# lukasvst/dm-vio

Hardware: NVIDIA H100
Metric: point-residuals/sec per GN iter (7 KF, 2000 pts, 640x480) (higher is better)
Workload: dtype f32

## Files before the change

### dm-vio_b200/capi.py

```python
import ctypes as C
import os

import numpy as np

_HERE = os.path.dirname(os.path.abspath(__file__))
LIB_PATH = os.environ.get("DMVIO_B200_LIB") or os.path.join(_HERE, "libdmvio_b200.so")
_LIB = None

f32p = np.ctypeslib.ndpointer(dtype=np.float32, flags="C_CONTIGUOUS")
f64p = np.ctypeslib.ndpointer(dtype=np.float64, flags="C_CONTIGUOUS")
i32p = np.ctypeslib.ndpointer(dtype=np.int32, flags="C_CONTIGUOUS")
vp = C.c_void_p

MAX_FRAMES = 8
PRECALC_FLOATS = 32


class DmvError(RuntimeError):
    pass


class BAConfig(C.Structure):
    _fields_ = [("w", C.c_int), ("h", C.c_int), ("max_frames", C.c_int), ("max_points", C.c_int), ("device", C.c_int), ("chunk_points", C.c_int)]


class BAParams(C.Structure):
    _fields_ = [("huberTH", C.c_float), ("outlierTHSumComponent", C.c_float), ("affineOptModeA", C.c_float), ("affineOptModeB", C.c_float)]


class BAState(C.Structure):
    _fields_ = [("calib", C.c_float * 8), ("precalc", vp), ("frameEnergyTH", vp), ("idepth", vp), ("idepth_zero", vp)]


class BALinResult(C.Structure):
    _fields_ = [("energy", C.c_double), ("n_in", C.c_int), ("n_oob", C.c_int), ("n_outlier", C.c_int)]


class BAActivateArgs(C.Structure):
    _fields_ = [("n", C.c_int)] + [(k, C.c_void_p) for k in ("host", "u", "v", "color8", "weights8", "energyTH", "idepth_min", "idepth_max", "RT")] + \
               [("minObs", C.c_int)] + [(k, C.c_void_p) for k in ("status", "idepth", "res_state")]


class BAMargArgs(C.Structure):
    _fields_ = [("n", C.c_int32), ("point", C.c_void_p), ("adHTdeltaF", C.c_void_p), ("cDeltaF", C.c_float * 4), ("idepthFixPriorMargFac", C.c_float)] + \
               [(k, C.c_void_p) for k in ("M", "Mb", "Msc", "Mbsc", "resInM", "ngoodRes", "res_toZeroF", "isLinearized")]


class IPPoints(C.Structure):
    _fields_ = [("n", C.c_int)] + [(k, C.c_void_p) for k in ("u", "v", "color8", "weights8", "gradH4", "energyTH", "idepth_min", "idepth_max", "quality",
                                                              "lastTraceStatus", "lastTraceUV2", "lastTracePixelInterval")]


class BABatch:

    def __init__(self, bas):
        self.L = lib()
        self.bas = list(bas)
        n = len(self.bas)
        self._harr = (C.c_void_p * n)(*[b.h for b in self.bas])
        h = C.c_void_p()
        check(self.L.dmv_ba_batch_create(self._harr, n, C.byref(h)))
        self.h = h

    def _args(self, xs, states):
        n = len(self.bas)
        self._xs = [None if x is None else _c(x, np.float64) for x in (xs or [None] * n)]
        self._sts = [b._state(*st) for b, st in zip(self.bas, states)]
        xarr = (C.c_void_p * n)(*[None if x is None else x.ctypes.data for x in self._xs])
        sarr = (C.c_void_p * n)(*[C.addressof(st) for st in self._sts])
        return xarr, sarr

    def gn_step(self, xs, states):
        n = len(self.bas)
        xarr, sarr = self._args(xs, states)
        res = (BALinResult * n)()
        sums = np.zeros(3 * n)
        check(self.L.dmv_ba_batch_gn_step(self.h, xarr, sarr, res, sums.ctypes.data))
        return [dict(energy=r.energy, n_in=r.n_in, n_oob=r.n_oob, n_outlier=r.n_outlier, sums=sums[3 * i:3 * i + 3]) for i, r in enumerate(res)]

    def bench(self, xs, states, iters=100, warmup=5):
        n = len(self.bas)
        xarr, sarr = self._args(xs, states)
        e2e, ker = C.c_double(0), C.c_double(0)
        check(self.L.dmv_ba_batch_bench(self.h, self._harr, n, xarr, sarr, max(1, warmup), C.byref(e2e), C.byref(ker)))
        check(self.L.dmv_ba_batch_bench(self.h, self._harr, n, xarr, sarr, iters, C.byref(e2e), C.byref(ker)))
        return ker.value, e2e.value, None

    def close(self):
        if self.h:
            self.L.dmv_ba_batch_destroy(self.h)
            self.h = None

    def __del__(self):
        try:
            self.close()
        except Exception:
            pass


class CTConfig(C.Structure):
    _fields_ = [("w", C.c_int), ("h", C.c_int), ("levels", C.c_int), ("max_points", C.c_int), ("device", C.c_int)]


class CIEvalArgs(C.Structure):
    _fields_ = [("level", C.c_int), ("RKi", C.c_float * 9), ("t_d", C.c_double * 3), ("t_log", C.c_double * 3), ("r2new_aff", C.c_float * 2),
                ("huberTH", C.c_float), ("alphaK", C.c_float), ("alphaW", C.c_float), ("couplingWeight", C.c_float),
                ("weightZeroPriorX", C.c_double), ("weightZeroPriorY", C.c_double),
                ("idepth_new", C.c_void_p), ("isGood", C.c_void_p), ("energy2", C.c_void_p), ("iR", C.c_void_p),
                ("isGood_new", C.c_void_p), ("energy_new2", C.c_void_p), ("maxstep", C.c_void_p), ("lastHessian_new", C.c_void_p),
                ("JbBuffer_new10", C.c_void_p)]


class CIEvalResult(C.Structure):
    _fields_ = [("H", C.c_float * 64), ("b", C.c_float * 8), ("Hsc", C.c_float * 64), ("bsc", C.c_float * 8), ("res3", C.c_float * 3),
                ("alphaOpt", C.c_float), ("n_good_new", C.c_int)]


SYMBOLS = [
    "dmv_last_error", "dmv_version", "dmv_device_count",
    "dmv_ba_create", "dmv_ba_destroy", "dmv_ba_set_params", "dmv_ba_default_params", "dmv_ba_upload_frame", "dmv_ba_upload_image", "dmv_ba_adopt_frame",
    "dmv_ba_set_window", "dmv_ba_set_points", "dmv_ba_set_residuals", "dmv_ba_set_adjoints", "dmv_ba_set_state", "dmv_ba_linearize",
    "dmv_ba_get_residual_outputs", "dmv_ba_get_target_energies", "dmv_ba_apply_res", "dmv_ba_accumulate", "dmv_ba_get_point_outputs", "dmv_ba_get_solve_HdiF",
    "dmv_ba_resubstitute", "dmv_ba_backup_points", "dmv_ba_restore_points", "dmv_ba_get_idepth", "dmv_ba_gn_step", "dmv_nccl_unique_id",
    "dmv_ba_comm_init", "dmv_ba_activate_points", "dmv_ba_marginalize_points", "dmv_ba_drop_residuals", "dmv_ba_reset_oob", "dmv_ba_p2p_export", "dmv_ba_p2p_import", "dmv_ba_last_timing", "dmv_ba_bench_device", "dmv_ba_kernel_launch_count", "dmv_ba_io_bytes", "dmv_ba_set_timing", "dmv_ba_bench_e2e",
    "dmv_ba_batch_create", "dmv_ba_batch_destroy", "dmv_ba_batch_gn_step", "dmv_ba_batch_set_timing", "dmv_ba_batch_last_kernel_ms", "dmv_ba_batch_bench",
    "dmv_ct_create", "dmv_ct_destroy", "dmv_ct_set_K", "dmv_ct_set_ref", "dmv_ct_make_coarse_depth", "dmv_ct_get_ref", "dmv_ct_upload_new", "dmv_ct_upload_new_image", "dmv_ct_set_huber",
    "dmv_ci_create", "dmv_ci_destroy", "dmv_ci_set_K", "dmv_ci_upload_first", "dmv_ci_upload_new", "dmv_ci_set_points", "dmv_ci_calc_res_and_gs", "dmv_ci_kernel_launch_count",
    "dmv_ct_calc_res_gs", "dmv_ct_track", "dmv_ip_default_settings", "dmv_ct_init_points", "dmv_ct_trace_points", "dmv_ct_trace_points_multi", "dmv_ct_set_timing", "dmv_ct_last_timing", "dmv_ct_kernel_launch_count", "dmv_ct_last_point_evaluations",
]


def lib():
    global _LIB
    if _LIB is None:
        if not os.path.exists(LIB_PATH):
            raise DmvError(f"{LIB_PATH} is missing: build it with `make -C dm-vio_b200` (python -c 'import __graft_entry__ as g; g.build()')")
        L = C.CDLL(LIB_PATH)
        L.dmv_last_error.restype = C.c_char_p
        L.dmv_version.restype = C.c_char_p
        L.dmv_ba_create.argtypes = [C.POINTER(BAConfig), C.POINTER(vp)]
        L.dmv_ba_destroy.argtypes = [vp]
        L.dmv_ba_set_params.argtypes = [vp, C.POINTER(BAParams)]
        L.dmv_ba_default_params.argtypes = [C.POINTER(BAParams)]
        L.dmv_ba_upload_frame.argtypes = [vp, C.c_int, f32p]
        L.dmv_ba_upload_image.argtypes = [vp, C.c_int, f32p]
        L.dmv_ba_set_window.argtypes = [vp, C.c_int, vp]
        L.dmv_ba_set_points.argtypes = [vp, C.c_int, i32p, f32p, f32p, f32p, vp, f32p, f32p, vp]
        L.dmv_ba_set_residuals.argtypes = [vp, C.c_int, i32p, i32p, vp, vp]
        L.dmv_ba_set_adjoints.argtypes = [vp, f64p, f64p]
        L.dmv_ba_set_state.argtypes = [vp, C.POINTER(BAState)]
        L.dmv_ba_linearize.argtypes = [vp, C.POINTER(BALinResult)]
        L.dmv_ba_get_residual_outputs.argtypes = [vp, vp, vp, vp, vp, vp]
        L.dmv_ba_get_target_energies.argtypes = [vp, C.c_int, f32p, C.c_int, C.POINTER(C.c_int)]
        L.dmv_ba_apply_res.argtypes = [vp]
        L.dmv_ba_accumulate.argtypes = [vp, f64p, f64p, f64p, f64p, C.POINTER(C.c_int)]
        L.dmv_ba_get_point_outputs.argtypes = [vp, vp, vp, vp, vp, vp]
        L.dmv_ba_resubstitute.argtypes = [vp, f64p, vp, C.c_int, f64p]
        L.dmv_ba_backup_points.argtypes = [vp]
        L.dmv_ba_restore_points.argtypes = [vp]
        L.dmv_ba_get_idepth.argtypes = [vp, vp, vp]
        L.dmv_ba_gn_step.argtypes = [vp, vp, C.POINTER(BAState), C.POINTER(BALinResult), f64p]
        L.dmv_nccl_unique_id.argtypes = [vp]
        L.dmv_ba_comm_init.argtypes = [vp, C.c_int, C.c_int, vp]
        L.dmv_ba_activate_points.argtypes = [vp, C.POINTER(BAActivateArgs)]
        L.dmv_ba_marginalize_points.argtypes = [vp, C.POINTER(BAMargArgs)]
        L.dmv_ba_drop_residuals.argtypes = [vp, C.c_int, i32p]
        L.dmv_ba_reset_oob.argtypes = [vp]
        L.dmv_ba_p2p_export.argtypes = [vp, vp]
        L.dmv_ba_p2p_import.argtypes = [vp, C.c_int, C.c_int, vp]
        L.dmv_ba_last_timing.argtypes = [vp, f32p]
        L.dmv_ba_bench_device.argtypes = [vp, vp, C.c_int, C.c_int, C.POINTER(C.c_float), C.POINTER(C.c_float)]
        L.dmv_ba_kernel_launch_count.argtypes = [vp, C.POINTER(C.c_longlong)]
        L.dmv_ba_set_timing.argtypes = [vp, C.c_int]
        L.dmv_ba_bench_e2e.argtypes = [vp, vp, C.POINTER(BAState), C.c_int, C.POINTER(C.c_double)]
        L.dmv_ba_io_bytes.argtypes = [vp, C.POINTER(C.c_longlong), C.POINTER(C.c_longlong)]
        L.dmv_ba_get_solve_HdiF.argtypes = [vp, f32p]
        L.dmv_ba_adopt_frame.argtypes = [vp, C.c_int, vp]
        L.dmv_ba_batch_create.argtypes = [vp, C.c_int, C.POINTER(vp)]
        L.dmv_ba_batch_destroy.argtypes = [vp]
        L.dmv_ba_batch_gn_step.argtypes = [vp, vp, vp, vp, vp]
        L.dmv_ba_batch_set_timing.argtypes = [vp, C.c_int]
        L.dmv_ba_batch_last_kernel_ms.argtypes = [vp, C.POINTER(C.c_float)]
        L.dmv_ba_batch_bench.argtypes = [vp, vp, C.c_int, vp, vp, C.c_int, C.POINTER(C.c_double), C.POINTER(C.c_double)]
        L.dmv_ct_create.argtypes = [C.POINTER(CTConfig), C.POINTER(vp)]
        L.dmv_ct_destroy.argtypes = [vp]
        L.dmv_ct_set_K.argtypes = [vp, C.c_int, C.c_float, C.c_float, C.c_float, C.c_float]
        L.dmv_ct_set_ref.argtypes = [vp, C.c_int, C.c_int, f32p, f32p, f32p, f32p]
        L.dmv_ct_make_coarse_depth.argtypes = [vp, C.c_int, f32p, f32p, f32p, f32p, i32p]
        L.dmv_ct_get_ref.argtypes = [vp, C.c_int, C.POINTER(C.c_int), vp, vp, vp, vp]
        L.dmv_ct_upload_new.argtypes = [vp, C.c_int, f32p]
        L.dmv_ct_upload_new_image.argtypes = [vp, f32p]
        L.dmv_ct_set_huber.argtypes = [vp, C.c_float]
        L.dmv_ct_calc_res_gs.argtypes = [vp, C.c_int, f32p, f32p, f32p, C.c_float, C.c_float, C.c_int, f64p, f64p, f64p, C.POINTER(C.c_int)]
        L.dmv_ct_init_points.argtypes = [vp, C.c_int, i32p, i32p, f32p, f32p, f32p, f32p, i32p]
        L.dmv_ct_trace_points.argtypes = [vp, C.POINTER(IPPoints), f32p, f32p, f32p, vp]
        L.dmv_ct_trace_points_multi.argtypes = [vp, C.c_int, vp, f32p, vp]
        L.dmv_ct_set_timing.argtypes = [vp, C.c_int]
        L.dmv_ct_last_timing.argtypes = [vp, f32p]
        L.dmv_ct_kernel_launch_count.argtypes = [vp, C.POINTER(C.c_longlong)]
        L.dmv_ct_last_point_evaluations.argtypes = [vp, C.POINTER(C.c_double)]
        L.dmv_ci_create.argtypes = [C.POINTER(CTConfig), C.POINTER(vp)]
        L.dmv_ci_destroy.argtypes = [vp]
        L.dmv_ci_set_K.argtypes = [vp, C.c_int, C.c_float, C.c_float, C.c_float, C.c_float]
        L.dmv_ci_upload_first.argtypes = [vp, C.c_int, vp]
        L.dmv_ci_upload_new.argtypes = [vp, C.c_int, vp]
        L.dmv_ci_set_points.argtypes = [vp, C.c_int, C.c_int, vp, vp, vp]
        L.dmv_ci_calc_res_and_gs.argtypes = [vp, C.POINTER(CIEvalArgs), C.POINTER(CIEvalResult)]
        L.dmv_ci_kernel_launch_count.argtypes = [vp, C.POINTER(C.c_longlong)]
        _LIB = L
    return _LIB


def check(rc):
    if rc != 0:
        raise DmvError(f"dmvio_b200 error {rc}: {lib().dmv_last_error().decode()}")


def _p(a):
    return None if a is None else a.ctypes.data_as(vp)


def _c(a, t):
    return None if a is None else np.ascontiguousarray(a, t)


class BA:

    def __init__(self, w, h, max_frames=8, max_points=8192, device=0, chunk_points=0):
        self.L = lib()
        cfg = BAConfig(w, h, max_frames, max_points, device, chunk_points)
        self.h = vp()
        check(self.L.dmv_ba_create(C.byref(cfg), C.byref(self.h)))
        self.w, self.hh = w, h
        self.nf = self.npts = self.nres = 0
        self._keep = {}

    def close(self):
        if self.h:
            self.L.dmv_ba_destroy(self.h)
            self.h = vp()

    def __del__(self):
        try:
            self.close()
        except Exception:
            pass

    def set_params(self, huberTH=9.0, outlierTHSumComponent=2500.0, affineOptModeA=1e12, affineOptModeB=1e8):
        p = BAParams(huberTH, outlierTHSumComponent, affineOptModeA, affineOptModeB)
        check(self.L.dmv_ba_set_params(self.h, C.byref(p)))

    def upload_frame(self, slot, dI):
        check(self.L.dmv_ba_upload_frame(self.h, slot, _c(dI, np.float32).reshape(-1)))

    def upload_image(self, slot, img):
        check(self.L.dmv_ba_upload_image(self.h, slot, _c(img, np.float32).reshape(-1)))

    def adopt_frame(self, slot, ct):
        check(self.L.dmv_ba_adopt_frame(self.h, slot, ct.h))

    def set_window(self, nf, slots=None):
        s = _c(slots, np.int32)
        check(self.L.dmv_ba_set_window(self.h, nf, _p(s)))
        self.nf = nf
        self.N = 8 * nf + 4

    def set_points(self, host, u, v, idepth, idepth_zero, color, weights, priorF=None):
        self.npts = len(host)
        iz, pf = _c(idepth_zero, np.float32), _c(priorF, np.float32)
        check(self.L.dmv_ba_set_points(self.h, self.npts, _c(host, np.int32), _c(u, np.float32), _c(v, np.float32), _c(idepth, np.float32),
                                       _p(iz), _c(color, np.float32).reshape(-1), _c(weights, np.float32).reshape(-1), _p(pf)))

    def set_residuals(self, point, target, state=None, energy=None):
        self.nres = len(point)
        s, e = _c(state, np.int32), _c(energy, np.float32)
        check(self.L.dmv_ba_set_residuals(self.h, self.nres, _c(point, np.int32), _c(target, np.int32), _p(s), _p(e)))

    def set_adjoints(self, adHost, adTarget):
        check(self.L.dmv_ba_set_adjoints(self.h, _c(adHost, np.float64).reshape(-1), _c(adTarget, np.float64).reshape(-1)))

    def _state(self, calib8, precalc, TH, idepth=None, idepth_zero=None):
        st = BAState()
        k = _c(calib8, np.float32)
        for i in range(8):
            st.calib[i] = float(k[i])
        pc, th, idd, idz = _c(precalc, np.float32), _c(TH, np.float32), _c(idepth, np.float32), _c(idepth_zero, np.float32)
        self._keep = dict(pc=pc, th=th, idd=idd, idz=idz)
        st.precalc, st.frameEnergyTH, st.idepth, st.idepth_zero = _p(pc), _p(th), _p(idd), _p(idz)
        return st

    def set_state(self, calib8, precalc, TH, idepth=None, idepth_zero=None):
        st = self._state(calib8, precalc, TH, idepth, idepth_zero)
        check(self.L.dmv_ba_set_state(self.h, C.byref(st)))

    def linearize(self):
        r = BALinResult()
        check(self.L.dmv_ba_linearize(self.h, C.byref(r)))
        return dict(energy=r.energy, n_in=r.n_in, n_oob=r.n_oob, n_outlier=r.n_outlier)

    def gn_step(self, x, calib8, precalc, TH, idepth=None, idepth_zero=None):
        st = self._state(calib8, precalc, TH, idepth, idepth_zero)
        r = BALinResult()
        sums = np.zeros(3)
        xx = _c(x, np.float64)
        check(self.L.dmv_ba_gn_step(self.h, _p(xx), C.byref(st), C.byref(r), sums))
        return dict(energy=r.energy, n_in=r.n_in, n_oob=r.n_oob, n_outlier=r.n_outlier, sums=sums)

    def residual_outputs(self):
        n = self.nres
        o = dict(newState=np.zeros(n, np.int32), newEnergy=np.zeros(n, np.float32), newEnergyWithOutlier=np.zeros(n, np.float32),
                 centerProjectedTo=np.zeros((n, 3), np.float32), JpJdF=np.zeros((n, 8), np.float32))
        check(self.L.dmv_ba_get_residual_outputs(self.h, _p(o["newState"]), _p(o["newEnergy"]), _p(o["newEnergyWithOutlier"]),
                                                 _p(o["centerProjectedTo"]), _p(o["JpJdF"])))
        return o

    def target_energies(self, target):
        out = np.zeros(max(self.npts, 1), np.float32)
        n = C.c_int(0)
        check(self.L.dmv_ba_get_target_energies(self.h, target, out, len(out), C.byref(n)))
        return out[:n.value]

    def apply_res(self):
        check(self.L.dmv_ba_apply_res(self.h))

    def accumulate(self):
        N = self.N
        o = dict(HA=np.zeros((N, N)), bA=np.zeros(N), Hsc=np.zeros((N, N)), bsc=np.zeros(N))
        n = C.c_int(0)
        check(self.L.dmv_ba_accumulate(self.h, o["HA"].reshape(-1), o["bA"], o["Hsc"].reshape(-1), o["bsc"], C.byref(n)))
        o["resInA"] = n.value
        return o

    def point_outputs(self):
        n = self.npts
        o = dict(Hdd=np.zeros(n, np.float32), bd=np.zeros(n, np.float32), Hcd=np.zeros((n, 4), np.float32), HdiF=np.zeros(n, np.float32),
                 bdSumF=np.zeros(n, np.float32))
        check(self.L.dmv_ba_get_point_outputs(self.h, _p(o["Hdd"]), _p(o["bd"]), _p(o["Hcd"]), _p(o["HdiF"]), _p(o["bdSumF"])))
        return o

    def resubstitute(self, x, apply=False):
        step = np.zeros(self.npts, np.float32)
        sums = np.zeros(3)
        check(self.L.dmv_ba_resubstitute(self.h, _c(x, np.float64), _p(step), int(apply), sums))
        return step, sums

    def backup_points(self):
        check(self.L.dmv_ba_backup_points(self.h))

    def restore_points(self):
        check(self.L.dmv_ba_restore_points(self.h))

    def get_idepth(self):
        a, b = np.zeros(self.npts, np.float32), np.zeros(self.npts, np.float32)
        check(self.L.dmv_ba_get_idepth(self.h, _p(a), _p(b)))
        return a, b

    def last_timing(self):
        ms = np.zeros(4, np.float32)
        check(self.L.dmv_ba_last_timing(self.h, ms))
        return ms

    def bench_device(self, x=None, iters=100, flush_l2=True):
        a, b = C.c_float(0), C.c_float(0)
        xx = _c(x, np.float64)
        check(self.L.dmv_ba_bench_device(self.h, _p(xx), iters, int(flush_l2), C.byref(a), C.byref(b)))
        return a.value, b.value

    def launch_count(self):
        n = C.c_longlong(0)
        check(self.L.dmv_ba_kernel_launch_count(self.h, C.byref(n)))
        return n.value

    def set_timing(self, enable=True):
        check(self.L.dmv_ba_set_timing(self.h, int(enable)))

    def bench_e2e(self, x, calib8, precalc, TH, iters=100):
        st = self._state(calib8, precalc, TH)
        ms = C.c_double(0)
        xx = _c(x, np.float64)
        check(self.L.dmv_ba_bench_e2e(self.h, _p(xx), C.byref(st), iters, C.byref(ms)))
        return ms.value

    def io_bytes(self):
        a, b = C.c_longlong(0), C.c_longlong(0)
        check(self.L.dmv_ba_io_bytes(self.h, C.byref(a), C.byref(b)))
        return a.value, b.value

    def comm_init(self, nranks, rank, uid_bytes):
        buf = C.create_string_buffer(bytes(uid_bytes), 128)
        check(self.L.dmv_ba_comm_init(self.h, nranks, rank, C.cast(buf, vp)))


    def activate_points(self, host, P, RT, minObs=1):
        n = len(P["u"])
        keep = [_c(host, np.int32)] + [_c(P[k], np.float32) for k in ("u", "v", "color", "weights", "energyTH", "idepth_min", "idepth_max")] + [_c(RT, np.float32)]
        status = np.zeros(n, np.int32); idepth = np.zeros(n, np.float32); rs = np.zeros((n, self.nf), np.int32)
        args = BAActivateArgs(n, *[a.ctypes.data for a in keep], int(minObs), status.ctypes.data, idepth.ctypes.data, rs.ctypes.data)
        check(self.L.dmv_ba_activate_points(self.h, C.byref(args)))
        return status, idepth, rs

    def reset_oob(self):
        check(self.L.dmv_ba_reset_oob(self.h))

    def drop_residuals(self, idx):
        idx = _c(idx, np.int32)
        check(self.L.dmv_ba_drop_residuals(self.h, len(idx), idx))
        self.nres -= len(np.unique(idx))

    def marginalize_points(self, pts, adHTdeltaF, cDeltaF, prior_fac=600.0 * 600.0):
        N = 8 * self.nf + 4
        pts = _c(pts, np.int32)
        ad = _c(adHTdeltaF, np.float32)
        assert ad.size == self.nf * self.nf * 8
        o = dict(M=np.zeros((N, N)), Mb=np.zeros(N), Msc=np.zeros((N, N)), Mbsc=np.zeros(N), ngood=np.zeros(len(pts), np.int32),
                 rtz=np.zeros((self.nres, 8), np.float32), isLinearized=np.zeros(self.nres, np.uint8))
        n = C.c_int32(0)
        args = BAMargArgs(len(pts), pts.ctypes.data, ad.ctypes.data, (C.c_float * 4)(*[float(x) for x in cDeltaF]), float(prior_fac),
                          o["M"].ctypes.data, o["Mb"].ctypes.data, o["Msc"].ctypes.data, o["Mbsc"].ctypes.data, C.addressof(n),
                          o["ngood"].ctypes.data, o["rtz"].ctypes.data, o["isLinearized"].ctypes.data)
        check(self.L.dmv_ba_marginalize_points(self.h, C.byref(args)))
        o["resInM"] = n.value
        o["H"], o["b"] = o["M"] - o["Msc"], o["Mb"] - o["Mbsc"]
        return o

    def p2p_export(self):
        buf = C.create_string_buffer(64)
        check(self.L.dmv_ba_p2p_export(self.h, C.cast(buf, vp)))
        return bytes(buf.raw)

    def p2p_import(self, nranks, rank, handles):
        blob = b"".join(bytes(h) for h in handles)
        assert len(blob) == 64 * nranks
        buf = C.create_string_buffer(blob, len(blob))
        check(self.L.dmv_ba_p2p_import(self.h, nranks, rank, C.cast(buf, vp)))


def nccl_unique_id():
    buf = C.create_string_buffer(128)
    check(lib().dmv_nccl_unique_id(C.cast(buf, vp)))
    return bytes(buf.raw)


class CT:
    def __init__(self, w, h, levels, max_points=65536, device=0):
        self.L = lib()
        cfg = CTConfig(w, h, levels, max_points, device)
        self.h = vp()
        check(self.L.dmv_ct_create(C.byref(cfg), C.byref(self.h)))
        self.levels = levels

    def close(self):
        if self.h:
            self.L.dmv_ct_destroy(self.h)
            self.h = vp()

    def __del__(self):
        try:
            self.close()
        except Exception:
            pass

    def set_K(self, lvl, fx, fy, cx, cy):
        check(self.L.dmv_ct_set_K(self.h, lvl, fx, fy, cx, cy))

    def set_ref(self, lvl, u, v, idepth, color):
        check(self.L.dmv_ct_set_ref(self.h, lvl, len(u), _c(u, np.float32), _c(v, np.float32), _c(idepth, np.float32), _c(color, np.float32)))

    def upload_new(self, lvl, dIp):
        check(self.L.dmv_ct_upload_new(self.h, lvl, _c(dIp, np.float32).reshape(-1)))

    def upload_new_image(self, img):
        check(self.L.dmv_ct_upload_new_image(self.h, _c(img, np.float32).reshape(-1)))

    def set_huber(self, th):
        check(self.L.dmv_ct_set_huber(self.h, th))

    def calc_res_gs(self, lvl, RKi, t, affLL, b0, cutoff, want_gs=True):
        res6 = np.zeros(6); H = np.zeros(64); b = np.zeros(8); n = C.c_int(0)
        check(self.L.dmv_ct_calc_res_gs(self.h, lvl, _c(RKi, np.float32).reshape(-1), _c(t, np.float32), _c(affLL, np.float32), b0, cutoff,
                                        int(want_gs), res6, H, b, C.byref(n)))
        return res6, H.reshape(8, 8), b, n.value

    def make_coarse_depth(self, Ku, Kv, new_idepth, HdiF):
        pc_n = np.zeros(8, np.int32)
        check(self.L.dmv_ct_make_coarse_depth(self.h, len(Ku), _c(Ku, np.float32), _c(Kv, np.float32), _c(new_idepth, np.float32), _c(HdiF, np.float32), pc_n))
        return pc_n

    def get_ref(self, lvl):
        n = C.c_int(0)
        check(self.L.dmv_ct_get_ref(self.h, lvl, C.byref(n), None, None, None, None))
        a = [np.zeros(n.value, np.float32) for _ in range(4)]
        check(self.L.dmv_ct_get_ref(self.h, lvl, C.byref(n), *[x.ctypes.data for x in a]))
        return dict(u=a[0], v=a[1], idepth=a[2], color=a[3])

    def init_points(self, u, v):
        n = len(u)
        P = dict(u=_c(u, np.float32), v=_c(v, np.float32), color=np.zeros((n, 8), np.float32), weights=np.zeros((n, 8), np.float32),
                 gradH=np.zeros((n, 4), np.float32), energyTH=np.zeros(n, np.float32))
        ok = np.zeros(n, np.int32)
        check(self.L.dmv_ct_init_points(self.h, n, _c(u, np.int32), _c(v, np.int32), P["color"].reshape(-1), P["weights"].reshape(-1), P["gradH"].reshape(-1),
                                        P["energyTH"], ok))
        P["ok"] = ok.astype(np.uint8)
        P.update(idepth_min=np.zeros(n, np.float32), idepth_max=np.full(n, np.nan, np.float32), quality=np.full(n, 10000, np.float32),
                 status=np.full(n, 5, np.int32), lastTraceUV=np.zeros((n, 2), np.float32), lastTracePixelInterval=np.zeros(n, np.float32))
        return P

    def trace_points(self, P, KRKi, Kt, aff):
        n = len(P["u"])
        keep = {k: _c(P[k], np.float32) for k in ("u", "v", "color", "weights", "gradH", "energyTH")}
        out = {"idepth_min": np.array(P["idepth_min"], np.float32, copy=True), "idepth_max": np.array(P["idepth_max"], np.float32, copy=True),
               "quality": np.array(P["quality"], np.float32, copy=True), "status": np.array(P["status"], np.int32, copy=True),
               "lastTraceUV": np.array(P["lastTraceUV"], np.float32, copy=True), "lastTracePixelInterval": np.array(P["lastTracePixelInterval"], np.float32, copy=True)}
        pts = IPPoints(n, *[a.ctypes.data for a in (keep["u"], keep["v"], keep["color"], keep["weights"], keep["gradH"], keep["energyTH"], out["idepth_min"],
                                                     out["idepth_max"], out["quality"], out["status"], out["lastTraceUV"], out["lastTracePixelInterval"])])
        check(self.L.dmv_ct_trace_points(self.h, C.byref(pts), _c(KRKi, np.float32).reshape(-1), _c(Kt, np.float32), _c(aff, np.float32), None))
        Q = dict(P)
        Q.update(out)
        return Q

    def trace_points_multi(self, sets):
        ns = len(sets)
        arr = (IPPoints * ns)()
        keeps, outs = [], []
        tab = np.zeros((ns, 14), np.float32)
        for k, (P, KRKi, Kt, aff) in enumerate(sets):
            keep = {q: _c(P[q], np.float32) for q in ("u", "v", "color", "weights", "gradH", "energyTH")}
            out = {"idepth_min": np.array(P["idepth_min"], np.float32, copy=True), "idepth_max": np.array(P["idepth_max"], np.float32, copy=True),
                   "quality": np.array(P["quality"], np.float32, copy=True), "status": np.array(P["status"], np.int32, copy=True),
                   "lastTraceUV": np.array(P["lastTraceUV"], np.float32, copy=True), "lastTracePixelInterval": np.array(P["lastTracePixelInterval"], np.float32, copy=True)}
            arr[k] = IPPoints(len(P["u"]), *[a.ctypes.data for a in (keep["u"], keep["v"], keep["color"], keep["weights"], keep["gradH"], keep["energyTH"], out["idepth_min"],
                                                                      out["idepth_max"], out["quality"], out["status"], out["lastTraceUV"], out["lastTracePixelInterval"])])
            tab[k, :9] = np.asarray(KRKi, np.float32).reshape(-1); tab[k, 9:12] = Kt; tab[k, 12:14] = aff
            keeps.append(keep); outs.append(out)
        check(self.L.dmv_ct_trace_points_multi(self.h, ns, C.addressof(arr), tab.reshape(-1), None))
        res = []
        for (P, _, _, _), out in zip(sets, outs):
            Q = dict(P); Q.update(out); res.append(Q)
        return res

    def set_timing(self, enable=True):
        check(self.L.dmv_ct_set_timing(self.h, int(enable)))

    def last_timing(self):
        ms = np.zeros(4, np.float32)
        check(self.L.dmv_ct_last_timing(self.h, ms))
        return ms

    def launch_count(self):
        n = C.c_longlong(0)
        check(self.L.dmv_ct_kernel_launch_count(self.h, C.byref(n)))
        return n.value


class CI:

    def __init__(self, w, h, levels, max_points=16384, device=0):
        self.L = lib()
        cfg = CTConfig(w, h, levels, max_points, device)
        self.h = vp()
        check(self.L.dmv_ci_create(C.byref(cfg), C.byref(self.h)))
        self.levels = levels

    def close(self):
        if self.h:
            self.L.dmv_ci_destroy(self.h)
            self.h = vp()

    def __del__(self):
        try:
            self.close()
        except Exception:
            pass

    def set_K(self, lvl, fx, fy, cx, cy):
        check(self.L.dmv_ci_set_K(self.h, lvl, C.c_float(fx), C.c_float(fy), C.c_float(cx), C.c_float(cy)))

    def upload_first(self, lvl, dIp):
        check(self.L.dmv_ci_upload_first(self.h, lvl, _p(_c(dIp, np.float32).reshape(-1))))

    def upload_new(self, lvl, dIp):
        check(self.L.dmv_ci_upload_new(self.h, lvl, _p(_c(dIp, np.float32).reshape(-1))))

    def set_points(self, lvl, u, v, outlierTH):
        check(self.L.dmv_ci_set_points(self.h, lvl, len(u), _p(_c(u, np.float32)), _p(_c(v, np.float32)), _p(_c(outlierTH, np.float32))))
        self._n = getattr(self, "_n", {})
        self._n[lvl] = len(u)

    def calc_res_and_gs(self, lvl, RKi, t, t_log, r2new_aff, idepth_new, isGood, energy2, iR, huberTH=9.0, alphaK=2.5 * 2.5, alphaW=150.0 * 150.0,
                        couplingWeight=1.0, wzpx=0.0, wzpy=0.0):
        n = self._n[lvl]
        a = CIEvalArgs()
        a.level = lvl
        a.RKi[:] = [float(x) for x in np.asarray(RKi, np.float32).reshape(-1)]
        a.t_d[:] = [float(x) for x in t]
        a.t_log[:] = [float(x) for x in t_log]
        a.r2new_aff[:] = [float(np.float32(x)) for x in r2new_aff]
        a.huberTH, a.alphaK, a.alphaW, a.couplingWeight, a.weightZeroPriorX, a.weightZeroPriorY = huberTH, alphaK, alphaW, couplingWeight, wzpx, wzpy
        ins = [_c(idepth_new, np.float32), _c(isGood, np.uint8), _c(energy2, np.float32).reshape(-1), _c(iR, np.float32)]
        a.idepth_new, a.isGood, a.energy2, a.iR = [x.ctypes.data for x in ins]
        o = dict(isGood_new=np.zeros(n, np.uint8), energy_new=np.zeros((n, 2), np.float32), maxstep=np.zeros(n, np.float32),
                 lastHessian_new=np.zeros(n, np.float32), Jb=np.zeros((n, 10), np.float32))
        a.isGood_new, a.energy_new2, a.maxstep, a.lastHessian_new, a.JbBuffer_new10 = [o[k].ctypes.data for k in ("isGood_new", "energy_new", "maxstep", "lastHessian_new", "Jb")]
        r = CIEvalResult()
        check(self.L.dmv_ci_calc_res_and_gs(self.h, C.byref(a), C.byref(r)))
        o.update(H=np.array(r.H, np.float32).reshape(8, 8), b=np.array(r.b, np.float32), Hsc=np.array(r.Hsc, np.float32).reshape(8, 8),
                 bsc=np.array(r.bsc, np.float32), res=np.array(r.res3, np.float32), alphaOpt=float(r.alphaOpt), n_good_new=int(r.n_good_new))
        return o
```

### dm-vio_b200/csrc/ba_bench.cu

```cuda
#include "../../include/dmvio_b200_bench.h"
#include "ba_handle.h"
#include <chrono>

using namespace dmv;

extern "C" {

int dmv_ba_bench_device(dmv_ba* b, const double* x, int iters, int flush_l2, float* ms_per_iter, float* ms_kernel) {
  int rc = dmv_ba_check_ready(b);
  if (rc != DMV_OK) return rc;
  if (iters < 1 || iters > 4096) return set_error(DMV_ERR_INVALID, "iters out of range");
  if (x && !b->have_committed) return set_error(DMV_ERR_STATE, "no committed linearisation to resubstitute");
  CK(cudaSetDevice(b->device));
  if (flush_l2 && !b->d_flush) {
    b->flush_n = (size_t)256 * 1024 * 1024 / sizeof(float4);
    CK(cudaMalloc(&b->d_flush, b->flush_n * sizeof(float4)));
    CK(cudaMemset(b->d_flush, 0, b->flush_n * sizeof(float4)));
  }
  if (x) dmv_ba_stage_x(b, x); else b->h_up->it.have_x = 0;
  std::vector<cudaEvent_t> e(3 * (size_t)iters);
  for (auto& ev : e) CK(cudaEventCreate(&ev));
  for (int i = 0; i < iters; i++) {
    if (flush_l2) launch_l2_flush(b->d_flush, b->flush_n, b->stream);
    dmv_ba_fill_descriptor(b);
    dmv_ba_next_exchange(b);
    HostUpload& U = *b->h_up;
    CK(cudaEventRecord(e[3 * i], b->stream));
    CK(launch_fused_kernel(U.win, U.it, false, b->stream, &b->bar_count));
    CK(cudaEventRecord(e[3 * i + 1], b->stream));
    if (b->nccl_comm && !b->xchg_on) {
      rc = dmv_ba_enqueue_exchange(b);
      if (rc != DMV_OK) return rc;
      CK(cudaEventRecord(e[3 * i + 2], b->stream));
    }
    b->launches += 1;
  }
  CK(cudaGetLastError());
  CK(cudaStreamSynchronize(b->stream));
  double tot = 0, pk = 0;
  for (int i = 0; i < iters; i++) {
    float a = 0, c = 0;
    cudaEventElapsedTime(&c, e[3 * i], e[3 * i + 1]);
    if (b->nccl_comm && !b->xchg_on) cudaEventElapsedTime(&a, e[3 * i], e[3 * i + 2]);
    else a = c;
    tot += a; pk += c;
  }
  for (auto& ev : e) cudaEventDestroy(ev);
  if (ms_per_iter) *ms_per_iter = (float)(tot / iters);
  if (ms_kernel) *ms_kernel = (float)(pk / iters);
  b->h_up->it.have_x = 0;
  b->have_tentative = true;
  return DMV_OK;
}

int dmv_ba_bench_e2e(dmv_ba* b, const double* x, const dmv_ba_state* st, int iters, double* ms_per_iter) {
  if (!b || !st || !ms_per_iter || iters < 1) return set_error(DMV_ERR_INVALID, "bad argument");
  dmv_ba_lin_result r;
  double sums[3];
  CK(cudaSetDevice(b->device));
  CK(cudaStreamSynchronize(b->stream));
  const auto t0 = std::chrono::steady_clock::now();
  for (int i = 0; i < iters; i++) {
    int rc = dmv_ba_gn_step(b, x, st, &r, sums);
    if (rc != DMV_OK) return rc;
    rc = dmv_ba_apply_res(b);
    if (rc != DMV_OK) return rc;
  }
  const auto t1 = std::chrono::steady_clock::now();
  *ms_per_iter = std::chrono::duration<double, std::milli>(t1 - t0).count() / iters;
  return DMV_OK;
}

int dmv_ba_batch_bench(dmv_ba_batch* B, dmv_ba* const* handles, int n, const double* const* x, const dmv_ba_state* const* st, int iters, double* e2e_ms_per_iter,
                       double* kernel_ms_per_iter) {
  if (!B || !handles || !st || iters < 1) return set_error(DMV_ERR_INVALID, "bad argument");
  int rc = dmv_ba_batch_set_timing(B, 1);
  if (rc != DMV_OK) return rc;
  double ksum = 0;
  const auto t0 = std::chrono::steady_clock::now();
  for (int i = 0; i < iters; i++) {
    rc = dmv_ba_batch_gn_step(B, x, st, nullptr, nullptr);
    if (rc != DMV_OK) return rc;
    for (int k = 0; k < n; k++) {
      rc = dmv_ba_apply_res(handles[k]);
      if (rc != DMV_OK) return rc;
    }
    float ms = 0.f;
    dmv_ba_batch_last_kernel_ms(B, &ms);
    ksum += ms;
  }
  const auto t1 = std::chrono::steady_clock::now();
  if (e2e_ms_per_iter) *e2e_ms_per_iter = std::chrono::duration<double, std::milli>(t1 - t0).count() / iters;
  if (kernel_ms_per_iter) *kernel_ms_per_iter = ksum / iters;
  return dmv_ba_batch_set_timing(B, 0);
}

}
```

### dm-vio_b200/csrc/ba_device.cuh

```cuda
#pragma once
#include <cuda_runtime.h>
#include <stdint.h>

namespace dmv {

constexpr int MAXF = 8;
constexpr int TOP_ROWS = 10;
constexpr int TOP_COLS = 13;
constexpr int TOP_TRI = 85;
constexpr int TOP_USED = TOP_TRI + 6;
constexpr int TOP_PART = 92;
__host__ __device__ constexpr int top_off(int r) { return r * TOP_COLS - (r * (r - 1)) / 2; }
constexpr int RES_NONE = 255, RES_IN = 0, RES_OOB = 1, RES_OUTLIER = 2;
constexpr int ACC_MISC = 8;
constexpr int PART_SLOT = 168;
constexpr int PART_CC = MAXF * PART_SLOT;
constexpr int PART_MISC = PART_CC + 20;
constexpr int PART_STRIDE = PART_MISC + ACC_MISC;

struct BAIter {
  float calib[8];
  float TH[MAXF];
  float precalc[MAXF * MAXF][32];
  float xAd[MAXF * MAXF][8];
  float xc[4];
  int have_x;
  int pad[3];
};

struct BAAdj {
  float adHostF[MAXF * MAXF][64];
  float adTdiagF[MAXF * MAXF][8];
  double adHost[MAXF * MAXF][64];
  double adTdiag[MAXF * MAXF][8];
};

constexpr int XCHG_MAXR = 8;
struct BAXchg {
  int nranks, rank, pitch;
  unsigned int seq;
  uint4* inbox[XCHG_MAXR];
};

struct BAMarg {
  float adHTdelta[MAXF * MAXF][8];
  float cDelta[4];
  float priorFac;
  int pad[3];
};

struct BAWinDev {
  int nf, npts, nchunks, w, h, N, NW, T, ntiles, mp, P;
  float huberTH, outlierTHSum;
  int zeroA, zeroB;
  int host_start[MAXF + 1];
  int chunk_beg[MAXF + 1];
  const float4* img[MAXF];
  const BAAdj* adj;
  const float2* uv;
  const float* idepth;
  const float* idepth_zero;
  const float* idepth_backup;
  float* idepth_out;
  const float* color;
  const float* weights;
  const float* priorF;
  const uint8_t* st_in;
  const float* en_in;
  uint8_t* st_new;
  float* en_new;
  float* en_wo;
  float* en_wo_newest_host;
  float* cpt;
  float* jpjd;
  float* pout;
  const uint8_t* c_st;
  const float* c_jpjd;
  const float* c_pout;
  float* step;
  double* part;
  float4* wg;
  float* hdig;
  unsigned int* bar;
  unsigned int bar_target;
  double* result;
  double* result_host;
  BAXchg xc;
  const BAMarg* marg;
  const uint8_t* marg_mask;
  float* marg_rtz;
};

constexpr int BATCH_MAX = 64;
struct BABatchHdr {
  int B, total;
  int prefix[BATCH_MAX + 1];
  unsigned int* bar;
  unsigned int bar_target;
};

inline __host__ __device__ int result_doubles(int N, int ntiles) { return N * N + N + ntiles * 16 + ACC_MISC; }

}
```

### dm-vio_b200/csrc/ba_fused.cu

```cuda
#include "ba_common.cuh"
#include <cstdlib>
#include <mutex>
#include <type_traits>

namespace dmv {

template <int K, int END, class F>
__device__ __forceinline__ void static_for(F&& f) {
  if constexpr (K < END) {
    f(std::integral_constant<int, K>{});
    static_for<K + 1, END>(f);
  }
}
__host__ __device__ constexpr int top_row(int k) {
  int r = 0;
  while (r < 9 && k >= top_off(r + 1)) r++;
  return r;
}
__host__ __device__ constexpr int top_col(int k) { return top_row(k) + k - top_off(top_row(k)); }

struct PixSums {
  float JI00, JI10, JI11, JabJI00, JabJI01, JabJI10, JabJI11, Jab00, Jab01, Jab11, JIr0, JIr1, Jabr0, Jabr1, rr;
};

template <int K>
__device__ __forceinline__ float top_entry(const float (&x)[10], const float (&y)[10], const float (&al)[10], const float (&be)[10], const PixSums& s) {
  if constexpr (K < TOP_TRI) {
    constexpr int r = top_row(K), c = top_col(K);
    if constexpr (c < 10) return al[r] * x[c] + be[r] * y[c];
    else if constexpr (c == 10) return x[r] * s.JabJI00 + y[r] * s.JabJI01;
    else if constexpr (c == 11) return x[r] * s.JabJI10 + y[r] * s.JabJI11;
    else return x[r] * s.JIr0 + y[r] * s.JIr1;
  } else if constexpr (K == TOP_TRI) return s.Jab00;
  else if constexpr (K == TOP_TRI + 1) return s.Jab01;
  else if constexpr (K == TOP_TRI + 2) return s.Jabr0;
  else if constexpr (K == TOP_TRI + 3) return s.Jab11;
  else if constexpr (K == TOP_TRI + 4) return s.Jabr1;
  else if constexpr (K == TOP_TRI + 5) return s.rr;
  else return 0.f;
}

template <int NH>
__device__ __forceinline__ float h13f(const float (*S)[96], int r, int c) {
  if (r > c) { const int t = r; r = c; c = t; }
  int idx;
  if (r < TOP_ROWS) idx = top_off(r) + c - r;
  else { const int rr = r - 10, cc = c - 10; idx = TOP_TRI + (rr == 0 ? cc : (rr == 1 ? 2 + cc : 5)); }
  if constexpr (NH == 2) return S[0][idx] + S[1][idx];
  else return S[0][idx];
}

__device__ __forceinline__ void geo_jac(const float* pc, float Kl0, float Kl1, float cu, float cv, float drescale, float new_idepth, float fx,
                                        float fy, float fxi, float fyi, float (&x)[10], float (&y)[10], float& ddx, float& ddy) {
  const float dCx2 = drescale * (pc[18] * cu - pc[12]);
  const float dCx3 = fx * drescale * (pc[19] * cu - pc[13]) * fyi;
  const float dCy2 = fy * drescale * (pc[18] * cv - pc[15]) * fxi;
  const float dCy3 = drescale * (pc[19] * cv - pc[16]);
  x[0] = (Kl0 * dCx2 + cu) * 50.0f; x[1] = (Kl1 * dCx3) * 50.0f; x[2] = (dCx2 + 1.f) * 50.0f; x[3] = dCx3 * 50.0f;
  y[0] = (Kl0 * dCy2) * 50.0f; y[1] = (Kl1 * dCy3 + cv) * 50.0f; y[2] = dCy2 * 50.0f; y[3] = (dCy3 + 1.f) * 50.0f;
  x[4] = new_idepth * fx; x[5] = 0.f; x[6] = -new_idepth * cu * fx; x[7] = -cu * cv * fx; x[8] = (1.f + cu * cu) * fx; x[9] = -cv * fx;
  y[4] = 0.f; y[5] = new_idepth * fy; y[6] = -new_idepth * cv * fy; y[7] = -(1.f + cv * cv) * fy; y[8] = cu * cv * fy; y[9] = cu * fy;
  ddx = drescale * (pc[21] - pc[23] * cu) * fx;
  ddy = drescale * (pc[22] - pc[23] * cv) * fy;
}

constexpr int OPS = 57;
template <int P, int LPR>
struct FusedSmem {
  static constexpr int NH = (LPR == 4) ? 2 : 1;
  double AhD[MAXF][64];
  double dT[MAXF][8];
  double G[MAXF][104];
  float adH[MAXF][64];
  float adT[MAXF][8];
  float pair[MAXF][NH][96];
  float rec[MAXF][16][P];
  float Wv[P][8 * MAXF + 8];
  float hdi[P];
  float id[P], idz[P];
  float misc[16][8];
  double red[16][32];
};

struct alignas(16) EntryTab { unsigned char v[96][4]; };
constexpr EntryTab make_entry_tab() {
  EntryTab t{};
  for (int k = 0; k < 96; k++) {
    if (k < TOP_TRI) {
      const int r = top_row(k), c = top_col(k);
      if (c < 10) { t.v[k][0] = 20 + r; t.v[k][1] = c; t.v[k][2] = 30 + r; t.v[k][3] = 10 + c; }
      else { t.v[k][0] = r; t.v[k][1] = 40 + 2 * (c - 10); t.v[k][2] = 10 + r; t.v[k][3] = 41 + 2 * (c - 10); }
    } else if (k < TOP_USED) { t.v[k][0] = 46 + (k - TOP_TRI); t.v[k][1] = 53; t.v[k][2] = 52; t.v[k][3] = 52; }
    else { t.v[k][0] = 52; t.v[k][1] = 52; t.v[k][2] = 52; t.v[k][3] = 52; }
  }
  return t;
}
static __device__ __constant__ EntryTab c_entry_tab = make_entry_tab();

__device__ __forceinline__ unsigned ld_acquire_u32(const unsigned* p) {
  unsigned v;
  asm volatile("ld.acquire.gpu.global.u32 %0, [%1];" : "=r"(v) : "l"(p) : "memory");
  return v;
}
__device__ __forceinline__ bool grid_barrier(unsigned* bar, unsigned target) {
  __shared__ int ok_s;
  __syncthreads();
  if (threadIdx.x == 0) {
    __threadfence();
    atomicAdd(bar, 1u);
    int ok = 1;
    const long long t0 = clock64();
    while ((int)(ld_acquire_u32(bar) - target) < 0) {
      if (clock64() - t0 > 200000000ll) { ok = 0; break; }
    }
    __threadfence();
    ok_s = ok;
  }
  __syncthreads();
  return ok_s != 0;
}

__device__ __forceinline__ void xchg_push(const BAXchg& X, int idx, double v) {
  const unsigned long long u = (unsigned long long)__double_as_longlong(v);
  const uint4 pk = make_uint4((unsigned)(u & 0xffffffffull), X.seq, (unsigned)(u >> 32), X.seq);
  const size_t off = (size_t)(((X.seq & 1u) * XCHG_MAXR + X.rank)) * X.pitch + idx;
#pragma unroll 1
  for (int k = 1; k < X.nranks; k++) {
    const int r = (X.rank + k) % X.nranks;
    uint4* dst = X.inbox[r] + off;
    asm volatile("st.volatile.global.v4.u32 [%0], {%1, %2, %3, %4};" ::"l"(dst), "r"(pk.x), "r"(pk.y), "r"(pk.z), "r"(pk.w) : "memory");
  }
}
constexpr long long XCHG_SPIN_LIMIT = 400000000ll;

__device__ __forceinline__ double xchg_pull_sum_lanes(const BAXchg& X, int idx, double mine, bool active, bool& ok) {
  const uint4* base = X.inbox[X.rank] + (size_t)((X.seq & 1u) * XCHG_MAXR) * X.pitch + idx;
  uint4 pk[XCHG_MAXR];
  unsigned pending = active ? (((1u << X.nranks) - 1u) & ~(1u << X.rank)) : 0u;
  const long long t0 = clock64();
  while (__any_sync(0xffffffffu, pending != 0u)) {
#pragma unroll
    for (int r = 0; r < XCHG_MAXR; r++)
      if ((pending >> r) & 1u) {
        const uint4* src = base + (size_t)r * X.pitch;
        asm volatile("ld.volatile.global.v4.u32 {%0, %1, %2, %3}, [%4];" : "=r"(pk[r].x), "=r"(pk[r].y), "=r"(pk[r].z), "=r"(pk[r].w) : "l"(src) : "memory");
      }
#pragma unroll
    for (int r = 0; r < XCHG_MAXR; r++)
      if (((pending >> r) & 1u) && pk[r].y == X.seq && pk[r].w == X.seq) pending &= ~(1u << r);
    if (__any_sync(0xffffffffu, clock64() - t0 > XCHG_SPIN_LIMIT)) break;
  }
  if (pending) { ok = false; return mine; }
  double s = 0.0;
#pragma unroll
  for (int r = 0; r < XCHG_MAXR; r++) {
    if (r >= X.nranks) break;
    s += (r == X.rank) ? mine : __longlong_as_double((long long)(((unsigned long long)pk[r].z << 32) | pk[r].x));
  }
  return active ? s : mine;
}

__device__ __forceinline__ double xchg_pull_sum_group(const BAXchg& X, int idx, double mine, bool active, bool& ok) {
  const int lane = threadIdx.x & 31, gl = lane & 15;
  const bool poll = active && gl < X.nranks && gl != X.rank;
  const uint4* src = X.inbox[X.rank] + (size_t)((X.seq & 1u) * XCHG_MAXR + (poll ? gl : 0)) * X.pitch + idx;
  uint4 pk = make_uint4(0u, 0u, 0u, 0u);
  bool pending = poll;
  const long long t0 = clock64();
  while (__any_sync(0xffffffffu, pending)) {
    if (pending) {
      asm volatile("ld.volatile.global.v4.u32 {%0, %1, %2, %3}, [%4];" : "=r"(pk.x), "=r"(pk.y), "=r"(pk.z), "=r"(pk.w) : "l"(src) : "memory");
      pending = !(pk.y == X.seq && pk.w == X.seq);
    }
    if (__any_sync(0xffffffffu, clock64() - t0 > XCHG_SPIN_LIMIT)) break;
  }
  if (__any_sync(0xffffffffu, pending)) ok = false;
  const double own = __shfl_sync(0xffffffffu, mine, lane & 16);
  const double v = (gl == X.rank) ? own : (poll ? __longlong_as_double((long long)(((unsigned long long)pk.z << 32) | pk.x)) : 0.0);
  double s = 0.0;
  for (int r = 0; r < X.nranks; r++) s += __shfl_sync(0xffffffffu, v, (lane & 16) | r);
  return s;
}

template <int P, int LPR, bool MARG>
__device__ __forceinline__ void fused_chunk(const BAWinDev& W, const BAIter& it, FusedSmem<P, LPR>& S, const int chunk) {
  constexpr int LOGP = (P == 32) ? 5 : 4;
  constexpr int NH = FusedSmem<P, LPR>::NH;
  const int nf = W.nf, N = W.N, mp = W.mp;
  const int tid = threadIdx.x, nthreads = blockDim.x;
  const int warp = tid >> 5, lane = tid & 31, nwarps = nthreads >> 5;
  const BAAdj* __restrict__ A = W.adj;
  int h = 0;
#pragma unroll
  for (int k = 1; k < MAXF; k++) h += (chunk >= W.chunk_beg[k]) ? 1 : 0;
  h = min(h, nf - 1);
  const int ch_start = W.host_start[h] + (chunk - W.chunk_beg[h]) * P;
  const int ch_count = min(P, W.host_start[h + 1] - ch_start);

  for (int i = tid; i < nf * 32; i += nthreads) cp_async16(&S.AhD[i >> 5][(i & 31) * 2], &A->adHost[h * nf + (i >> 5)][(i & 31) * 2]);
  for (int i = tid; i < nf * 4; i += nthreads) cp_async16(&S.dT[i >> 2][(i & 3) * 2], &A->adTdiag[h * nf + (i >> 2)][(i & 3) * 2]);
  asm volatile("cp.async.commit_group;" ::: "memory");

  float e_sum = 0.f, rs_step2 = 0.f, rs_nid = 0.f, rs_cnt = 0.f;
  int n_in = 0, n_oob = 0, n_outl = 0;
  if constexpr (LPR == 1) {
  const int r = tid >> LOGP, pl = tid & (P - 1);
  const int t = r + (r >= h ? 1 : 0);
  const bool slot_ok = r < nf - 1;
  {
    const int tc = slot_ok ? t : (h == 0 ? 1 : 0);
    if (slot_ok) {
      if (pl < 16) *reinterpret_cast<float4*>(&S.adH[t][pl * 4]) = __ldg(reinterpret_cast<const float4*>(&A->adHostF[h * nf + t][pl * 4]));
      if (pl < 2) *reinterpret_cast<float4*>(&S.adT[t][pl * 4]) = __ldg(reinterpret_cast<const float4*>(&A->adTdiagF[h * nf + t][pl * 4]));
    }
    const bool valid = slot_ok && pl < ch_count;
    const int p = ch_start + min(pl, ch_count - 1);
    const int slot = tc * mp + p;
    const float* pc = it.precalc[h * nf + tc];
    const float fx = it.calib[0], fy = it.calib[1], cx = it.calib[2], cy = it.calib[3];
    const float fxi = it.calib[4], fyi = it.calib[5];
    const float TH = fmaxf(it.TH[h], it.TH[tc]);
    const float wM3 = (float)(W.w - 3), hM3 = (float)(W.h - 3);
    const float4* __restrict__ img = W.img[tc];
    const int iw = W.w;
    const float huber = W.huberTH, oth = W.outlierTHSum;

    int st = valid ? (int)__ldg(W.st_in + slot) : RES_NONE;
    float en_old = __ldg(W.en_in + slot);
    bool masked = true;
    if constexpr (MARG) {
      masked = valid && __ldg(W.marg_mask + p) != 0;
      st = (masked && st != RES_NONE) ? RES_IN : RES_NONE;
      en_old = 0.f;
    }
    const float2 uv = __ldg(W.uv + p);
    float col[8], wgt[8];
    {
      const float4 c0 = __ldg(reinterpret_cast<const float4*>(W.color + (size_t)p * 8)), c1 = __ldg(reinterpret_cast<const float4*>(W.color + (size_t)p * 8) + 1);
      const float4 w0 = __ldg(reinterpret_cast<const float4*>(W.weights + (size_t)p * 8)), w1 = __ldg(reinterpret_cast<const float4*>(W.weights + (size_t)p * 8) + 1);
      col[0] = c0.x; col[1] = c0.y; col[2] = c0.z; col[3] = c0.w; col[4] = c1.x; col[5] = c1.y; col[6] = c1.z; col[7] = c1.w;
      wgt[0] = w0.x; wgt[1] = w0.y; wgt[2] = w0.z; wgt[3] = w0.w; wgt[4] = w1.x; wgt[5] = w1.y; wgt[6] = w1.z; wgt[7] = w1.w;
    }
    float idepth, idz;
    if (it.have_x) {
      const float4 po0 = __ldg(reinterpret_cast<const float4*>(W.c_pout + (size_t)p * 8));
      const float4 po1 = __ldg(reinterpret_cast<const float4*>(W.c_pout + (size_t)p * 8) + 1);
      const float idb = __ldg(W.idepth_backup + p);
      float b = po1.w - (it.xc[0] * po0.z + it.xc[1] * po0.w + it.xc[2] * po1.x + it.xc[3] * po1.y);
      int ngood = 0;
#pragma unroll
      for (int t4 = 0; t4 < MAXF; t4 += 4) {
        int stc[4];
        float4 a0[4], a1[4];
#pragma unroll
        for (int u = 0; u < 4; u++) {
          const int cs = min(t4 + u, nf - 1) * mp + p;
          stc[u] = __ldg(W.c_st + cs);
          a0[u] = __ldg(reinterpret_cast<const float4*>(W.c_jpjd + (size_t)cs * 8));
          a1[u] = __ldg(reinterpret_cast<const float4*>(W.c_jpjd + (size_t)cs * 8) + 1);
        }
#pragma unroll
        for (int u = 0; u < 4; u++) {
          const int tt = t4 + u;
          const bool good = tt < nf && tt != h && stc[u] == RES_IN;
          const float* xa = it.xAd[h * nf + min(tt, nf - 1)];
          const float dot = xa[0] * a0[u].x + xa[1] * a0[u].y + xa[2] * a0[u].z + xa[3] * a0[u].w + xa[4] * a1[u].x + xa[5] * a1[u].y + xa[6] * a1[u].z + xa[7] * a1[u].w;
          b -= good ? dot : 0.f;
          ngood += good;
        }
      }
      const float step = ngood > 0 ? -b * po1.z : 0.f;
      idepth = idb + step;
      idz = idepth;
      if (r == 0 && valid) {
        W.step[p] = step;
        W.idepth_out[p] = idepth;
        rs_step2 = step * step; rs_nid = fabsf(idb); rs_cnt = 1.f;
      }
    } else {
      idepth = __ldg(W.idepth + p);
      idz = __ldg(W.idepth_zero + p);
    }
    if (r == 0 && valid) { S.id[pl] = idepth; S.idz[pl] = idz; }
    bool live = (st != RES_NONE) && (st != RES_OOB);

    const float Kl0 = (uv.x - cx) * fxi, Kl1 = (uv.y - cy) * fyi;
    const float q2 = pc[18] * Kl0 + pc[19] * Kl1 + pc[20] + pc[23] * idz;
    const float drescale = 1.0f / q2;
    const float new_idepth = idz * drescale;
    const float cu = (pc[12] * Kl0 + pc[13] * Kl1 + pc[14] + pc[21] * idz) * drescale;
    const float cv = (pc[15] * Kl0 + pc[16] * Kl1 + pc[17] + pc[22] * idz) * drescale;
    const float cKu = cu * fx + cx, cKv = cv * fy + cy;
    live = live && (drescale > 0.f) && cKu > 1.1f && cKv > 1.1f && cKu < wM3 && cKv < hM3;

    float Ku[8], Kv[8];
#pragma unroll
    for (int j = 0; j < 8; j++) {
      const float pu = uv.x + (float)c_pattern[j][0], pv = uv.y + (float)c_pattern[j][1];
      const float r2 = pc[6] * pu + pc[7] * pv + pc[8] + pc[11] * idepth;
      Ku[j] = (pc[0] * pu + pc[1] * pv + pc[2] + pc[9] * idepth) / r2;
      Kv[j] = (pc[3] * pu + pc[4] * pv + pc[5] + pc[10] * idepth) / r2;
      live = live && Ku[j] > 1.1f && Kv[j] > 1.1f && Ku[j] < wM3 && Kv[j] < hM3;
    }
    float x[10], y[10], ddx = 0.f, ddy = 0.f, jpx = 0.f, jpy = 0.f, dp6 = 0.f, dp7 = 0.f;
    if constexpr (MARG) {
      if (live) {
        geo_jac(pc, Kl0, Kl1, cu, cv, drescale, new_idepth, fx, fy, fxi, fyi, x, y, ddx, ddy);
        const float* dp = W.marg->adHTdelta[h * nf + tc];
        const float* cD = W.marg->cDelta;
        const float dlt = idepth - idz;
        jpx = (x[4] * dp[0] + x[5] * dp[1] + x[6] * dp[2] + x[7] * dp[3] + x[8] * dp[4] + x[9] * dp[5]) +
              (x[0] * cD[0] + x[1] * cD[1] + x[2] * cD[2] + x[3] * cD[3]) + ddx * dlt;
        jpy = (y[4] * dp[0] + y[5] * dp[1] + y[6] * dp[2] + y[7] * dp[3] + y[8] * dp[4] + y[9] * dp[5]) +
              (y[0] * cD[0] + y[1] * cD[1] + y[2] * cD[2] + y[3] * cD[3]) + ddy * dlt;
        dp6 = dp[6]; dp7 = dp[7];
      }
    }

    PixSums s = {0.f, 0.f, 0.f, 0.f, 0.f, 0.f, 0.f, 0.f, 0.f, 0.f, 0.f, 0.f, 0.f, 0.f, 0.f};
    float energy = 0.f, wJI2 = 0.f, rtz[8];
    if (live) {
      const bool zA = W.zeroA != 0, zB = W.zeroB != 0;
#pragma unroll
      for (int half = 0; half < 2; half++) {
      float4 tap[4][4];
#pragma unroll
      for (int jj = 0; jj < 4; jj++) {
        const int j = half * 4 + jj;
        const int ix = (int)Ku[j], iy = (int)Kv[j];
        const float4* bp = img + (size_t)iy * iw + ix;
        tap[jj][0] = __ldg(bp); tap[jj][1] = __ldg(bp + 1); tap[jj][2] = __ldg(bp + iw); tap[jj][3] = __ldg(bp + iw + 1);
      }
#pragma unroll
      for (int jj = 0; jj < 4; jj++) {
        const int j = half * 4 + jj;
        const int ix = (int)Ku[j], iy = (int)Kv[j];
        const float dx = Ku[j] - ix, dy = Kv[j] - iy, dxdy = dx * dy;
        const float w11 = dxdy, w10 = dy - dxdy, w01 = dx - dxdy, w00 = 1 - dx - dy + dxdy;
        const float h0 = w11 * tap[jj][3].x + w10 * tap[jj][2].x + w01 * tap[jj][1].x + w00 * tap[jj][0].x;
        const float h1 = w11 * tap[jj][3].y + w10 * tap[jj][2].y + w01 * tap[jj][1].y + w00 * tap[jj][0].y;
        const float h2 = w11 * tap[jj][3].z + w10 * tap[jj][2].z + w01 * tap[jj][1].z + w00 * tap[jj][0].z;
        live = live && isfinite(h0);
        const float residual = h0 - (pc[24] * col[j] + pc[25]);
        const float drdA = col[j] - pc[26];
        float w = sqrtf(oth / (oth + (h1 * h1 + h2 * h2)));
        w = 0.5f * (w + wgt[j]);
        const float ar = fabsf(residual);
        float hw = ar < huber ? 1.f : huber / ar;
        energy += w * w * hw * residual * residual * (2.f - hw);
        if (hw < 1.f) hw = sqrtf(hw);
        hw = hw * w;
        const float gx = h1 * hw, gy = h2 * hw;
        const float resF = residual * hw;
        const float ja = drdA * hw, jb = hw;
        const float jaF = zA ? 0.f : ja, jbF = zB ? 0.f : jb;
        float ra = resF;
        if constexpr (MARG) { ra = (((resF - gx * jpx) - gy * jpy) - jaF * dp6) - jbF * dp7; rtz[j] = ra; }
        s.JI00 += gx * gx; s.JI11 += gy * gy; s.JI10 += gx * gy;
        s.JabJI00 += ja * gx; s.JabJI01 += ja * gy; s.JabJI10 += jb * gx; s.JabJI11 += jb * gy;
        s.Jab00 += ja * ja; s.Jab01 += ja * jb; s.Jab11 += jb * jb;
        s.JIr0 += ra * gx; s.JIr1 += ra * gy; s.Jabr0 += ra * jaF; s.Jabr1 += ra * jbF; s.rr += ra * ra;
        wJI2 += hw * hw * (gx * gx + gy * gy);
      }
      }
    }

    int newState;
    float newEnergy;
    if (st == RES_NONE) { newState = RES_NONE; newEnergy = 0.f; }
    else if (!live) { newState = RES_OOB; newEnergy = en_old; }
    else if (energy > TH || wJI2 < 2.f) { newState = RES_OUTLIER; newEnergy = TH; }
    else { newState = RES_IN; newEnergy = energy; }
    const bool in = (newState == RES_IN);
    if (st != RES_NONE) {
      e_sum = newEnergy;
      n_in = in; n_oob = (newState == RES_OOB); n_outl = (newState == RES_OUTLIER);
    }
    if constexpr (MARG) {
      if (masked) {
        float4* o = reinterpret_cast<float4*>(W.marg_rtz + (size_t)slot * 8);
        o[0] = in ? make_float4(rtz[0], rtz[1], rtz[2], rtz[3]) : make_float4(0.f, 0.f, 0.f, 0.f);
        o[1] = in ? make_float4(rtz[4], rtz[5], rtz[6], rtz[7]) : make_float4(0.f, 0.f, 0.f, 0.f);
      }
    }
    if (valid && masked) {
      W.st_new[slot] = (uint8_t)newState;
      W.en_new[slot] = newEnergy;
      const float ewo = (st == RES_NONE || !live) ? -1.f : energy;
      W.en_wo[slot] = ewo;
      if (tc == nf - 1 && W.en_wo_newest_host) W.en_wo_newest_host[p] = ewo;
      const size_t plane = (size_t)MAXF * mp;
      W.cpt[slot] = cKu; W.cpt[plane + slot] = cKv; W.cpt[2 * plane + slot] = new_idepth;
    }

    float jp[8] = {0.f, 0.f, 0.f, 0.f, 0.f, 0.f, 0.f, 0.f}, Hdd = 0.f, bd = 0.f, Hcd0 = 0.f, Hcd1 = 0.f, Hcd2 = 0.f, Hcd3 = 0.f;
    if (in) {
      if constexpr (!MARG) geo_jac(pc, Kl0, Kl1, cu, cv, drescale, new_idepth, fx, fy, fxi, fyi, x, y, ddx, ddy);
      const float J0 = s.JI00 * ddx + s.JI10 * ddy, J1 = s.JI10 * ddx + s.JI11 * ddy;
#pragma unroll
      for (int k = 0; k < 6; k++) jp[k] = x[4 + k] * J0 + y[4 + k] * J1;
      jp[6] = s.JabJI00 * ddx + s.JabJI01 * ddy; jp[7] = s.JabJI10 * ddx + s.JabJI11 * ddy;
      Hdd = J0 * ddx + J1 * ddy;
      bd = s.JIr0 * ddx + s.JIr1 * ddy;
      Hcd0 = x[0] * J0 + y[0] * J1; Hcd1 = x[1] * J0 + y[1] * J1; Hcd2 = x[2] * J0 + y[2] * J1; Hcd3 = x[3] * J0 + y[3] * J1;
      if (valid) {
        float4* gj = reinterpret_cast<float4*>(W.jpjd + (size_t)slot * 8);
        gj[0] = make_float4(jp[0], jp[1], jp[2], jp[3]);
        gj[1] = make_float4(jp[4], jp[5], jp[6], jp[7]);
      }
    } else {
#pragma unroll
      for (int k = 0; k < 10; k++) { x[k] = 0.f; y[k] = 0.f; }
      s = PixSums{0.f, 0.f, 0.f, 0.f, 0.f, 0.f, 0.f, 0.f, 0.f, 0.f, 0.f, 0.f, 0.f, 0.f, 0.f};
    }
    __syncwarp();
    if (slot_ok) {
#pragma unroll
      for (int k = 0; k < 8; k++) {
        const float4 a0 = *reinterpret_cast<const float4*>(&S.adH[t][k * 8]), a1 = *reinterpret_cast<const float4*>(&S.adH[t][k * 8 + 4]);
        S.rec[t][k][pl] = a0.x * jp[0] + a0.y * jp[1] + a0.z * jp[2] + a0.w * jp[3] + a1.x * jp[4] + a1.y * jp[5] + a1.z * jp[6] + a1.w * jp[7];
        S.Wv[pl][4 + 8 * t + k] = S.adT[t][k] * jp[k];
      }
      S.rec[t][8][pl] = Hdd; S.rec[t][9][pl] = bd; S.rec[t][10][pl] = Hcd0; S.rec[t][11][pl] = Hcd1; S.rec[t][12][pl] = Hcd2; S.rec[t][13][pl] = Hcd3;
      S.rec[t][14][pl] = in ? 1.f : 0.f;
    }

    float al[10], be[10];
#pragma unroll
    for (int k = 0; k < 10; k++) { al[k] = s.JI00 * x[k] + s.JI10 * y[k]; be[k] = s.JI10 * x[k] + s.JI11 * y[k]; }
    float v[48];
    {
      const bool up = (lane & (P / 2)) != 0;
      static_for<0, 48>([&](auto kc) {
        constexpr int k = decltype(kc)::value;
        const float a = top_entry<k>(x, y, al, be, s), b = top_entry<k + 48>(x, y, al, be, s);
        v[k] = (up ? b : a) + __shfl_xor_sync(0xffffffffu, up ? a : b, P / 2);
      });
    }
    static_for<0, LOGP - 1>([&](auto sc) {
      constexpr int st2 = decltype(sc)::value, hstep = 24 >> st2, m = (P / 4) >> st2;
      const bool up = (lane & m) != 0;
#pragma unroll
      for (int k = 0; k < hstep; k++) v[k] = (up ? v[k + hstep] : v[k]) + __shfl_xor_sync(0xffffffffu, up ? v[k] : v[k + hstep], m);
    });
    if (slot_ok) {
      constexpr int PER = 96 / P;
#pragma unroll
      for (int k = 0; k < PER; k++) S.pair[t][0][PER * pl + k] = v[k];
    }
  }
  } else {
  static_assert(LPR == 1 || P == 16, "LPR = 4 is written for chunks of 16 points");
  const int r = tid >> 6;
  const int pl = (tid & 63) >> 2, q = tid & 3;
  const int half = (tid >> 5) & 1;
  const bool pair_ok = r < nf - 1;
  const int t = pair_ok ? r + (r >= h ? 1 : 0) : (h == 0 ? 1 : 0);
  {
    const bool valid = pair_ok && pl < ch_count;
    const int p = ch_start + min(pl, ch_count - 1);
    const int slot = t * mp + p;
    const float* pc = it.precalc[h * nf + t];
    const float fx = it.calib[0], fy = it.calib[1], cx = it.calib[2], cy = it.calib[3];
    const float fxi = it.calib[4], fyi = it.calib[5];
    const float TH = fmaxf(it.TH[h], it.TH[t]);
    const float wM3 = (float)(W.w - 3), hM3 = (float)(W.h - 3);
    const float4* __restrict__ img = W.img[t];
    const int iw = W.w;
    const float huber = W.huberTH, oth = W.outlierTHSum;

    int st = valid ? (int)__ldg(W.st_in + slot) : RES_NONE;
    float en_old = __ldg(W.en_in + slot);
    bool masked = true;
    if constexpr (MARG) {
      masked = valid && __ldg(W.marg_mask + p) != 0;
      st = (masked && st != RES_NONE) ? RES_IN : RES_NONE;
      en_old = 0.f;
    }
    const float2 uv = __ldg(W.uv + p);
    const float2 col = __ldg(reinterpret_cast<const float2*>(W.color + (size_t)p * 8) + q);
    const float2 wgt = __ldg(reinterpret_cast<const float2*>(W.weights + (size_t)p * 8) + q);
    float4 ah[4];
#pragma unroll
    for (int u = 0; u < 4; u++) ah[u] = __ldg(reinterpret_cast<const float4*>(&A->adHostF[h * nf + t][q * 16]) + u);
    const float2 at2 = __ldg(reinterpret_cast<const float2*>(&A->adTdiagF[h * nf + t][q * 2]));
    float idepth, idz;
    if (it.have_x) {
      const float4 po0 = __ldg(reinterpret_cast<const float4*>(W.c_pout + (size_t)p * 8));
      const float4 po1 = __ldg(reinterpret_cast<const float4*>(W.c_pout + (size_t)p * 8) + 1);
      const float idb = __ldg(W.idepth_backup + p);
      float b = po1.w - (it.xc[0] * po0.z + it.xc[1] * po0.w + it.xc[2] * po1.x + it.xc[3] * po1.y);
      int ngood = 0;
#pragma unroll
      for (int t4 = 0; t4 < MAXF; t4 += 4) {
        int stc[4];
        float4 a0[4], a1[4];
#pragma unroll
        for (int u = 0; u < 4; u++) {
          const int cs = min(t4 + u, nf - 1) * mp + p;
          stc[u] = __ldg(W.c_st + cs);
          a0[u] = __ldg(reinterpret_cast<const float4*>(W.c_jpjd + (size_t)cs * 8));
          a1[u] = __ldg(reinterpret_cast<const float4*>(W.c_jpjd + (size_t)cs * 8) + 1);
        }
#pragma unroll
        for (int u = 0; u < 4; u++) {
          const int tt = t4 + u;
          const bool good = tt < nf && tt != h && stc[u] == RES_IN;
          const float* xa = it.xAd[h * nf + min(tt, nf - 1)];
          const float dot = xa[0] * a0[u].x + xa[1] * a0[u].y + xa[2] * a0[u].z + xa[3] * a0[u].w + xa[4] * a1[u].x + xa[5] * a1[u].y + xa[6] * a1[u].z + xa[7] * a1[u].w;
          b -= good ? dot : 0.f;
          ngood += good;
        }
      }
      const float step = ngood > 0 ? -b * po1.z : 0.f;
      idepth = idb + step;
      idz = idepth;
      if (r == 0 && q == 0 && valid) {
        W.step[p] = step;
        W.idepth_out[p] = idepth;
        rs_step2 = step * step; rs_nid = fabsf(idb); rs_cnt = 1.f;
      }
    } else {
      idepth = __ldg(W.idepth + p);
      idz = __ldg(W.idepth_zero + p);
    }
    if (r == 0 && q == 0 && valid) { S.id[pl] = idepth; S.idz[pl] = idz; }
    bool live = (st != RES_NONE) && (st != RES_OOB);

    const float Kl0 = (uv.x - cx) * fxi, Kl1 = (uv.y - cy) * fyi;
    const float q2 = pc[18] * Kl0 + pc[19] * Kl1 + pc[20] + pc[23] * idz;
    const float drescale = 1.0f / q2;
    const float new_idepth = idz * drescale;
    const float cu = (pc[12] * Kl0 + pc[13] * Kl1 + pc[14] + pc[21] * idz) * drescale;
    const float cv = (pc[15] * Kl0 + pc[16] * Kl1 + pc[17] + pc[22] * idz) * drescale;
    const float cKu = cu * fx + cx, cKv = cv * fy + cy;
    live = live && (drescale > 0.f) && cKu > 1.1f && cKv > 1.1f && cKu < wM3 && cKv < hM3;

    float Ku[2], Kv[2];
#pragma unroll
    for (int jj = 0; jj < 2; jj++) {
      const float pu = uv.x + (float)c_pattern[2 * q + jj][0], pv = uv.y + (float)c_pattern[2 * q + jj][1];
      const float r2 = pc[6] * pu + pc[7] * pv + pc[8] + pc[11] * idepth;
      Ku[jj] = (pc[0] * pu + pc[1] * pv + pc[2] + pc[9] * idepth) / r2;
      Kv[jj] = (pc[3] * pu + pc[4] * pv + pc[5] + pc[10] * idepth) / r2;
      live = live && Ku[jj] > 1.1f && Kv[jj] > 1.1f && Ku[jj] < wM3 && Kv[jj] < hM3;
    }
    {
      const unsigned bal = __ballot_sync(0xffffffffu, live);
      live = ((bal >> (lane & ~3)) & 0xfu) == 0xfu;
    }
    float x[10], y[10], ddx = 0.f, ddy = 0.f, jpx = 0.f, jpy = 0.f, dp6 = 0.f, dp7 = 0.f;
    if constexpr (MARG) {
      if (live) {
        geo_jac(pc, Kl0, Kl1, cu, cv, drescale, new_idepth, fx, fy, fxi, fyi, x, y, ddx, ddy);
        const float* dp = W.marg->adHTdelta[h * nf + t];
        const float* cD = W.marg->cDelta;
        const float dlt = idepth - idz;
        jpx = (x[4] * dp[0] + x[5] * dp[1] + x[6] * dp[2] + x[7] * dp[3] + x[8] * dp[4] + x[9] * dp[5]) +
              (x[0] * cD[0] + x[1] * cD[1] + x[2] * cD[2] + x[3] * cD[3]) + ddx * dlt;
        jpy = (y[4] * dp[0] + y[5] * dp[1] + y[6] * dp[2] + y[7] * dp[3] + y[8] * dp[4] + y[9] * dp[5]) +
              (y[0] * cD[0] + y[1] * cD[1] + y[2] * cD[2] + y[3] * cD[3]) + ddy * dlt;
        dp6 = dp[6]; dp7 = dp[7];
      }
    }

    float sv[17];
#pragma unroll
    for (int k = 0; k < 17; k++) sv[k] = 0.f;
    float rtz[2] = {0.f, 0.f};
    bool fin = true;
    if (live) {
      const bool zA = W.zeroA != 0, zB = W.zeroB != 0;
      float4 tap[2][4];
#pragma unroll
      for (int jj = 0; jj < 2; jj++) {
        const int ix = (int)Ku[jj], iy = (int)Kv[jj];
        const float4* bp = img + (size_t)iy * iw + ix;
        tap[jj][0] = __ldg(bp); tap[jj][1] = __ldg(bp + 1); tap[jj][2] = __ldg(bp + iw); tap[jj][3] = __ldg(bp + iw + 1);
      }
#pragma unroll
      for (int jj = 0; jj < 2; jj++) {
        const int ix = (int)Ku[jj], iy = (int)Kv[jj];
        const float dx = Ku[jj] - ix, dy = Kv[jj] - iy, dxdy = dx * dy;
        const float w11 = dxdy, w10 = dy - dxdy, w01 = dx - dxdy, w00 = 1 - dx - dy + dxdy;
        const float h0 = w11 * tap[jj][3].x + w10 * tap[jj][2].x + w01 * tap[jj][1].x + w00 * tap[jj][0].x;
        const float h1 = w11 * tap[jj][3].y + w10 * tap[jj][2].y + w01 * tap[jj][1].y + w00 * tap[jj][0].y;
        const float h2 = w11 * tap[jj][3].z + w10 * tap[jj][2].z + w01 * tap[jj][1].z + w00 * tap[jj][0].z;
        fin = fin && isfinite(h0);
        const float cj = jj ? col.y : col.x, wj = jj ? wgt.y : wgt.x;
        const float residual = h0 - (pc[24] * cj + pc[25]);
        const float drdA = cj - pc[26];
        float w = sqrtf(oth / (oth + (h1 * h1 + h2 * h2)));
        w = 0.5f * (w + wj);
        const float ar = fabsf(residual);
        float hw = ar < huber ? 1.f : huber / ar;
        sv[15] += w * w * hw * residual * residual * (2.f - hw);
        if (hw < 1.f) hw = sqrtf(hw);
        hw = hw * w;
        const float gx = h1 * hw, gy = h2 * hw;
        const float resF = residual * hw;
        const float ja = drdA * hw, jb = hw;
        const float jaF = zA ? 0.f : ja, jbF = zB ? 0.f : jb;
        float ra = resF;
        if constexpr (MARG) { ra = (((resF - gx * jpx) - gy * jpy) - jaF * dp6) - jbF * dp7; rtz[jj] = ra; }
        sv[0] += gx * gx; sv[2] += gy * gy; sv[1] += gx * gy;
        sv[3] += ja * gx; sv[4] += ja * gy; sv[5] += jb * gx; sv[6] += jb * gy;
        sv[7] += ja * ja; sv[8] += ja * jb; sv[9] += jb * jb;
        sv[10] += ra * gx; sv[11] += ra * gy; sv[12] += ra * jaF; sv[13] += ra * jbF; sv[14] += ra * ra;
        sv[16] += hw * hw * (gx * gx + gy * gy);
      }
    }
    {
      const unsigned bal = __ballot_sync(0xffffffffu, fin);
      live = live && (((bal >> (lane & ~3)) & 0xfu) == 0xfu);
#pragma unroll
      for (int k = 0; k < 17; k++) {
        sv[k] += __shfl_xor_sync(0xffffffffu, sv[k], 1);
        sv[k] += __shfl_xor_sync(0xffffffffu, sv[k], 2);
      }
    }
    PixSums s = {sv[0], sv[1], sv[2], sv[3], sv[4], sv[5], sv[6], sv[7], sv[8], sv[9], sv[10], sv[11], sv[12], sv[13], sv[14]};
    const float energy = sv[15], wJI2 = sv[16];

    int newState;
    float newEnergy;
    if (st == RES_NONE) { newState = RES_NONE; newEnergy = 0.f; }
    else if (!live) { newState = RES_OOB; newEnergy = en_old; }
    else if (energy > TH || wJI2 < 2.f) { newState = RES_OUTLIER; newEnergy = TH; }
    else { newState = RES_IN; newEnergy = energy; }
    const bool in = (newState == RES_IN);
    if (st != RES_NONE && q == 0) {
      e_sum = newEnergy;
      n_in = in; n_oob = (newState == RES_OOB); n_outl = (newState == RES_OUTLIER);
    }
    if constexpr (MARG) {
      if (masked) *reinterpret_cast<float2*>(W.marg_rtz + (size_t)slot * 8 + 2 * q) = in ? make_float2(rtz[0], rtz[1]) : make_float2(0.f, 0.f);
    }
    if (valid && masked && q == 0) {
      W.st_new[slot] = (uint8_t)newState;
      W.en_new[slot] = newEnergy;
      const float ewo = (st == RES_NONE || !live) ? -1.f : energy;
      W.en_wo[slot] = ewo;
      if (t == nf - 1 && W.en_wo_newest_host) W.en_wo_newest_host[p] = ewo;
      const size_t plane = (size_t)MAXF * mp;
      W.cpt[slot] = cKu; W.cpt[plane + slot] = cKv; W.cpt[2 * plane + slot] = new_idepth;
    }

    float jp[8] = {0.f, 0.f, 0.f, 0.f, 0.f, 0.f, 0.f, 0.f}, Hdd = 0.f, bd = 0.f, Hcd0 = 0.f, Hcd1 = 0.f, Hcd2 = 0.f, Hcd3 = 0.f;
    if (in) {
      if constexpr (!MARG) geo_jac(pc, Kl0, Kl1, cu, cv, drescale, new_idepth, fx, fy, fxi, fyi, x, y, ddx, ddy);
      const float J0 = s.JI00 * ddx + s.JI10 * ddy, J1 = s.JI10 * ddx + s.JI11 * ddy;
#pragma unroll
      for (int k = 0; k < 6; k++) jp[k] = x[4 + k] * J0 + y[4 + k] * J1;
      jp[6] = s.JabJI00 * ddx + s.JabJI01 * ddy; jp[7] = s.JabJI10 * ddx + s.JabJI11 * ddy;
      Hdd = J0 * ddx + J1 * ddy;
      bd = s.JIr0 * ddx + s.JIr1 * ddy;
      Hcd0 = x[0] * J0 + y[0] * J1; Hcd1 = x[1] * J0 + y[1] * J1; Hcd2 = x[2] * J0 + y[2] * J1; Hcd3 = x[3] * J0 + y[3] * J1;
      if (valid && q == 0) {
        float4* gj = reinterpret_cast<float4*>(W.jpjd + (size_t)slot * 8);
        gj[0] = make_float4(jp[0], jp[1], jp[2], jp[3]);
        gj[1] = make_float4(jp[4], jp[5], jp[6], jp[7]);
      }
    } else {
#pragma unroll
      for (int k = 0; k < 10; k++) { x[k] = 0.f; y[k] = 0.f; }
      s = PixSums{0.f, 0.f, 0.f, 0.f, 0.f, 0.f, 0.f, 0.f, 0.f, 0.f, 0.f, 0.f, 0.f, 0.f, 0.f};
    }
    {
      const float r0 = ah[0].x * jp[0] + ah[0].y * jp[1] + ah[0].z * jp[2] + ah[0].w * jp[3] + ah[1].x * jp[4] + ah[1].y * jp[5] + ah[1].z * jp[6] + ah[1].w * jp[7];
      const float r1 = ah[2].x * jp[0] + ah[2].y * jp[1] + ah[2].z * jp[2] + ah[2].w * jp[3] + ah[3].x * jp[4] + ah[3].y * jp[5] + ah[3].z * jp[6] + ah[3].w * jp[7];
      const float j0 = (q == 0) ? jp[0] : (q == 1) ? jp[2] : (q == 2) ? jp[4] : jp[6];
      const float j1 = (q == 0) ? jp[1] : (q == 1) ? jp[3] : (q == 2) ? jp[5] : jp[7];
      if (pair_ok) {
        S.rec[t][2 * q][pl] = r0; S.rec[t][2 * q + 1][pl] = r1;
        S.Wv[pl][4 + 8 * t + 2 * q] = at2.x * j0; S.Wv[pl][4 + 8 * t + 2 * q + 1] = at2.y * j1;
      }
      const float e0 = (q == 0) ? Hdd : (q == 1) ? Hcd0 : (q == 2) ? Hcd2 : (in ? 1.f : 0.f);
      const float e1 = (q == 0) ? bd : (q == 1) ? Hcd1 : (q == 2) ? Hcd3 : 0.f;
      const int k0 = (q == 0) ? 8 : (q == 1) ? 10 : (q == 2) ? 12 : 14;
      if (pair_ok) { S.rec[t][k0][pl] = e0; S.rec[t][k0 + 1][pl] = e1; }
    }

    float v[32];
    {
      const float alq[3] = {s.JI00 * ((q == 0) ? x[0] : (q == 1) ? x[1] : (q == 2) ? x[2] : x[3]) + s.JI10 * ((q == 0) ? y[0] : (q == 1) ? y[1] : (q == 2) ? y[2] : y[3]),
                            s.JI00 * ((q == 0) ? x[4] : (q == 1) ? x[5] : (q == 2) ? x[6] : x[7]) + s.JI10 * ((q == 0) ? y[4] : (q == 1) ? y[5] : (q == 2) ? y[6] : y[7]),
                            s.JI00 * ((q == 0) ? x[8] : (q == 1) ? x[9] : 0.f) + s.JI10 * ((q == 0) ? y[8] : (q == 1) ? y[9] : 0.f)};
      const float beq[3] = {s.JI10 * ((q == 0) ? x[0] : (q == 1) ? x[1] : (q == 2) ? x[2] : x[3]) + s.JI11 * ((q == 0) ? y[0] : (q == 1) ? y[1] : (q == 2) ? y[2] : y[3]),
                            s.JI10 * ((q == 0) ? x[4] : (q == 1) ? x[5] : (q == 2) ? x[6] : x[7]) + s.JI11 * ((q == 0) ? y[4] : (q == 1) ? y[5] : (q == 2) ? y[6] : y[7]),
                            s.JI10 * ((q == 0) ? x[8] : (q == 1) ? x[9] : 0.f) + s.JI11 * ((q == 0) ? y[8] : (q == 1) ? y[9] : 0.f)};
      const float xq[3] = {(q == 0) ? x[0] : (q == 1) ? x[1] : (q == 2) ? x[2] : x[3], (q == 0) ? x[4] : (q == 1) ? x[5] : (q == 2) ? x[6] : x[7],
                           (q == 0) ? x[8] : (q == 1) ? x[9] : 0.f};
      const float yq[3] = {(q == 0) ? y[0] : (q == 1) ? y[1] : (q == 2) ? y[2] : y[3], (q == 0) ? y[4] : (q == 1) ? y[5] : (q == 2) ? y[6] : y[7],
                           (q == 0) ? y[8] : (q == 1) ? y[9] : 0.f};
      int o = 0;
#pragma unroll
      for (int j = 0; j < 3; j++) {
#pragma unroll
        for (int c = 4 * j; c < 13; c++) {
          float val;
          if (c < 10) val = alq[j] * x[c] + beq[j] * y[c];
          else if (c == 10) val = xq[j] * s.JabJI00 + yq[j] * s.JabJI01;
          else if (c == 11) val = xq[j] * s.JabJI10 + yq[j] * s.JabJI11;
          else val = xq[j] * s.JIr0 + yq[j] * s.JIr1;
          v[o++] = val;
        }
      }
      if (q == 2) { v[22] = s.Jab00; v[23] = s.Jab01; v[24] = s.Jabr0; v[25] = s.Jab11; v[26] = s.Jabr1; }
      v[27] = (q == 2) ? s.rr : 0.f;
      if (q == 3) { v[22] = v[23] = v[24] = v[25] = v[26] = 0.f; }
      v[28] = v[29] = v[30] = v[31] = 0.f;
    }
    static_for<0, 3>([&](auto sc) {
      constexpr int st2 = decltype(sc)::value, hstep = 16 >> st2, m = 16 >> st2;
      const bool up = (lane & m) != 0;
#pragma unroll
      for (int k = 0; k < hstep; k++) v[k] = (up ? v[k + hstep] : v[k]) + __shfl_xor_sync(0xffffffffu, up ? v[k] : v[k + hstep], m);
    });
    if (pair_ok) {
      const int w8 = (lane >> 2) & 7;
#pragma unroll
      for (int k = 0; k < 4; k++) {
        const int pos = 4 * w8 + k;
        int idx = -1;
        if (pos < 13) { const int rr = q, c = pos; if (c >= rr) idx = top_off(rr) + c - rr; }
        else if (pos < 22) { const int rr = q + 4, c = pos - 13 + 4; if (c >= rr) idx = top_off(rr) + c - rr; }
        else if (pos < 28) {
          if (q < 2) { const int rr = q + 8, c = pos - 22 + 8; if (pos < 27 && c >= rr) idx = top_off(rr) + c - rr; }
          else if (q == 2) idx = TOP_TRI + (pos - 22);
        }
        if (idx >= 0) S.pair[t][half][idx] = v[k];
      }
    }
  }
  }
  {
    float es = e_sum, fin = (float)n_in, foob = (float)n_oob, fout = (float)n_outl;
#pragma unroll
    for (int m = 1; m < 32; m <<= 1) {
      es += __shfl_xor_sync(0xffffffffu, es, m);
      fin += __shfl_xor_sync(0xffffffffu, fin, m);
      foob += __shfl_xor_sync(0xffffffffu, foob, m);
      fout += __shfl_xor_sync(0xffffffffu, fout, m);
      rs_step2 += __shfl_xor_sync(0xffffffffu, rs_step2, m);
      rs_nid += __shfl_xor_sync(0xffffffffu, rs_nid, m);
      rs_cnt += __shfl_xor_sync(0xffffffffu, rs_cnt, m);
    }
    if (lane == 0) {
      S.misc[warp][0] = es; S.misc[warp][1] = fin; S.misc[warp][2] = foob; S.misc[warp][3] = fout;
      S.misc[warp][4] = rs_step2; S.misc[warp][5] = rs_nid; S.misc[warp][6] = rs_cnt; S.misc[warp][7] = 0.f;
    }
  }
  cp_async_wait_all();
  __syncthreads();

  for (int e = tid; e < ch_count * 9; e += nthreads) {
    const int k = e / ch_count, pl2 = e - k * ch_count;
    if (k < 8) {
      float sum = 0.f;
      for (int tt = 0; tt < nf; tt++)
        if (tt != h) sum += S.rec[tt][k][pl2];
      S.Wv[pl2][4 + 8 * h + k] = sum;
    } else {
      const int p = ch_start + pl2;
      float Hdd = 0.f, bd = 0.f, c0 = 0.f, c1 = 0.f, c2 = 0.f, c3 = 0.f, ngood = 0.f;
      for (int tt = 0; tt < nf; tt++) {
        if (tt == h) continue;
        Hdd += S.rec[tt][8][pl2]; bd += S.rec[tt][9][pl2]; c0 += S.rec[tt][10][pl2]; c1 += S.rec[tt][11][pl2];
        c2 += S.rec[tt][12][pl2]; c3 += S.rec[tt][13][pl2]; ngood += S.rec[tt][14][pl2];
      }
      float prior = __ldg(W.priorF + p);
      bool masked = true;
      if constexpr (MARG) { masked = __ldg(W.marg_mask + p) != 0; prior *= __ldg(&W.marg->priorFac); }
      float HdiF = 0.f, bdSum = 0.f, w0 = 0.f, w1 = 0.f, w2 = 0.f, w3 = 0.f;
      if (ngood > 0.f) {
        float H = Hdd + prior;
        if (H < 1e-10f) H = 1e-10f;
        HdiF = 1.0f / H;
        bdSum = MARG ? bd : bd + prior * (S.id[pl2] - S.idz[pl2]);
        w0 = c0; w1 = c1; w2 = c2; w3 = c3;
      }
      S.Wv[pl2][0] = w0; S.Wv[pl2][1] = w1; S.Wv[pl2][2] = w2; S.Wv[pl2][3] = w3;
      S.Wv[pl2][N] = bdSum;
      for (int c = N + 1; c < W.NW; c++) S.Wv[pl2][c] = 0.f;
      S.hdi[pl2] = HdiF;
      if (masked) {
        float4* po = reinterpret_cast<float4*>(W.pout + (size_t)p * 8);
        po[0] = make_float4(Hdd, bd, c0, c1);
        po[1] = make_float4(c2, c3, HdiF, bdSum);
      }
    }
  }
  for (int e = tid; e < nf * 104; e += nthreads) {
    const int tt = e / 104, rr = e - tt * 104, i = rr / 13, c = rr - i * 13;
    if (tt == h) continue;
    const int colc = (c < 8) ? 4 + c : (c < 12 ? c - 8 : 12);
    double m = 0.0;
#pragma unroll
    for (int k = 0; k < 8; k++) m += S.AhD[tt][i * 8 + k] * (double)h13f<NH>(S.pair[tt], 4 + k, colc);
    S.G[tt][rr] = m;
  }
  __syncthreads();

  {
    const int T = W.T;
    for (int e = tid; e < ch_count * T; e += nthreads) {
      const int g4 = e / ch_count, pl2 = e - g4 * ch_count;
      W.wg[(size_t)g4 * mp + ch_start + pl2] = *reinterpret_cast<const float4*>(&S.Wv[pl2][4 * g4]);
    }
    if (tid < ch_count) W.hdig[ch_start + tid] = S.hdi[tid];
  }
  {
    double* __restrict__ out = W.part + (size_t)chunk * PART_STRIDE;
    for (int e = tid; e < nf * PART_SLOT; e += nthreads) {
      const int tt = e / PART_SLOT, q = e - tt * PART_SLOT;
      double val;
      if (tt != h) {
        const float (*B)[96] = S.pair[tt];
        if (q < 64) { const int i = q >> 3, j = q & 7; val = S.G[tt][i * 13 + j] * S.dT[tt][j]; }
        else if (q < 128) { const int i = (q - 64) >> 3, j = q & 7; val = S.dT[tt][i] * (double)h13f<NH>(B, 4 + i, 4 + j) * S.dT[tt][j]; }
        else if (q < 160) { const int i = (q - 128) >> 2, c = q & 3; val = S.dT[tt][i] * (double)h13f<NH>(B, 4 + i, c); }
        else { const int i = q - 160; val = S.dT[tt][i] * (double)h13f<NH>(B, 4 + i, 12); }
      } else {
        if (q < 64) continue;
        val = 0.0;
        if (q < 128) {
          const int i = (q - 64) >> 3, j = q & 7;
          for (int t2 = 0; t2 < nf; t2++) {
            if (t2 == h) continue;
#pragma unroll
            for (int k = 0; k < 8; k++) val += S.G[t2][i * 13 + k] * S.AhD[t2][j * 8 + k];
          }
        } else if (q < 160) {
          const int i = (q - 128) >> 2, c = q & 3;
          for (int t2 = 0; t2 < nf; t2++) if (t2 != h) val += S.G[t2][i * 13 + 8 + c];
        } else {
          const int i = q - 160;
          for (int t2 = 0; t2 < nf; t2++) if (t2 != h) val += S.G[t2][i * 13 + 12];
        }
      }
      out[e] = val;
    }
    if (tid < 20) {
      const int i = tid / 5, j = tid - i * 5;
      double val = 0.0;
      for (int t2 = 0; t2 < nf; t2++) if (t2 != h) val += (double)h13f<NH>(S.pair[t2], i, j < 4 ? j : 12);
      out[PART_CC + (j < 4 ? i * 4 + j : 16 + i)] = val;
    } else if (tid >= 32 && tid < 40) {
      const int k = tid - 32;
      double val = 0.0;
      for (int wv = 0; wv < nwarps; wv++) val += (double)S.misc[wv][k];
      out[PART_MISC + k] = val;
    }
  }
  __syncthreads();
}

template <int P, int LPR>
__device__ __forceinline__ void fused_reduce(const BAWinDev& W, FusedSmem<P, LPR>& S, bool ok, const int vcta, const int ncta) {
  const int nf = W.nf, N = W.N, mp = W.mp;
  const int tid = threadIdx.x, nthreads = blockDim.x;
  const int warp = tid >> 5, lane = tid & 31, nwarps = nthreads >> 5;

  const int nH = N * N + N;
  double* __restrict__ R = W.result;
  double* __restrict__ RH = W.result_host;
  const bool xch = W.xc.nranks > 1;
  const double* __restrict__ part = W.part;

  const int npair = nf * (nf - 1) / 2;
  const int n_off = npair * 64, n_diag = nf * 64, n_c = nf * 32, n_b = nf * 8;
  const int nitems = n_off + n_diag + n_c + n_b + 16 + 4 + (ACC_MISC - 1);
  const int grp = tid >> 4, gl = tid & 15, groups_per_cta = nthreads >> 4;
  const int nch = W.nchunks;
  auto phase_d = [&](const int pass) {
    for (int base = vcta * groups_per_cta; base < nitems; base += ncta * groups_per_cta) {
      const int item = base + grp;
      const bool act = item < nitems;
      int off0 = 0, lo0 = 0, hi0 = act ? nch : 0, off1 = 0, lo1 = 0, hi1 = 0, d0 = 0, d1 = -1;
      int e = act ? item : nitems - 1;
      if (e < n_off) {
        const int q = e >> 6, ij = e & 63, i = ij >> 3, j = ij & 7;
        int a = 0, rem = q;
        while (rem >= nf - 1 - a) { rem -= nf - 1 - a; a++; }
        const int b = a + 1 + rem;
        off0 = b * PART_SLOT + i * 8 + j; lo0 = W.chunk_beg[a]; hi0 = act ? W.chunk_beg[a + 1] : lo0;
        off1 = a * PART_SLOT + j * 8 + i; lo1 = W.chunk_beg[b]; hi1 = act ? W.chunk_beg[b + 1] : lo1;
        d0 = (4 + 8 * a + i) * N + 4 + 8 * b + j; d1 = (4 + 8 * b + j) * N + 4 + 8 * a + i;
      } else if ((e -= n_off) < n_diag) {
        const int a = e >> 6, ij = e & 63;
        off0 = a * PART_SLOT + 64 + ij;
        d0 = (4 + 8 * a + (ij >> 3)) * N + 4 + 8 * a + (ij & 7);
      } else if ((e -= n_diag) < n_c) {
        const int a = e >> 5, ic = e & 31;
        off0 = a * PART_SLOT + 128 + ic;
        d0 = (4 + 8 * a + (ic >> 2)) * N + (ic & 3); d1 = (ic & 3) * N + 4 + 8 * a + (ic >> 2);
      } else if ((e -= n_c) < n_b) {
        off0 = (e >> 3) * PART_SLOT + 160 + (e & 7);
        d0 = N * N + 4 + e;
      } else if ((e -= n_b) < 16) {
        off0 = PART_CC + e; d0 = (e >> 2) * N + (e & 3);
      } else if ((e -= 16) < 4) {
        off0 = PART_CC + 16 + e; d0 = N * N + e;
      } else {
        e -= 4;
        off0 = PART_MISC + e; d0 = nH + W.ntiles * 16 + e;
      }
      if (pass == 0) {
        double sum = 0.0;
#pragma unroll 1
        for (int seg = 0; seg < 2; seg++) {
          const int lo = seg ? lo1 : lo0, hi = seg ? hi1 : hi0;
          const double* __restrict__ src = part + (seg ? off1 : off0);
          for (int c0 = lo + gl; c0 < hi; c0 += 192) {
            double v[12];
#pragma unroll
            for (int u = 0; u < 12; u++) v[u] = (c0 + 16 * u < hi) ? __ldcg(src + (size_t)(c0 + 16 * u) * PART_STRIDE) : 0.0;
#pragma unroll
            for (int u = 0; u < 12; u++) sum += v[u];
          }
        }
        sum += __shfl_xor_sync(0xffffffffu, sum, 8);
        sum += __shfl_xor_sync(0xffffffffu, sum, 4);
        sum += __shfl_xor_sync(0xffffffffu, sum, 2);
        sum += __shfl_xor_sync(0xffffffffu, sum, 1);
        if (gl == 0 && act) {
          if (xch) { R[d0] = sum; xchg_push(W.xc, d0, sum); }
          else { R[d0] = sum; if (d1 >= 0) R[d1] = sum; if (RH) { RH[d0] = sum; if (d1 >= 0) RH[d1] = sum; } }
        }
      } else {
        const double sum = xchg_pull_sum_group(W.xc, d0, (gl == 0 && act) ? R[d0] : 0.0, act, ok);
        if (gl == 0 && act) {
          R[d0] = sum; if (d1 >= 0) R[d1] = sum;
          if (RH) { RH[d0] = sum; if (d1 >= 0) RH[d1] = sum; }
        }
      }
    }
    };
  phase_d(0);

  {
    const int T = W.T, npts = W.npts;
    for (int tile0 = vcta; tile0 < W.ntiles; tile0 += 2 * ncta) {
      const int tile1 = tile0 + ncta;
      const bool two = tile1 < W.ntiles;
      int ti0 = 0, rem = tile0;
      while (rem >= T - ti0) { rem -= T - ti0; ti0++; }
      const int tj0 = ti0 + rem;
      int ti1 = 0;
      rem = two ? tile1 : tile0;
      while (rem >= T - ti1) { rem -= T - ti1; ti1++; }
      const int tj1 = ti1 + rem;
      float a[2][4][4];
#pragma unroll
      for (int q = 0; q < 2; q++)
#pragma unroll
        for (int i = 0; i < 4; i++)
#pragma unroll
          for (int j = 0; j < 4; j++) a[q][i][j] = 0.f;
      const float4* __restrict__ wi0 = W.wg + (size_t)ti0 * mp;
      const float4* __restrict__ wj0 = W.wg + (size_t)tj0 * mp;
      const float4* __restrict__ wi1 = W.wg + (size_t)ti1 * mp;
      const float4* __restrict__ wj1 = W.wg + (size_t)tj1 * mp;
#pragma unroll 4
      for (int p = tid; p < npts; p += nthreads) {
        const float sc = __ldcg(W.hdig + p);
        const float4 wi = __ldcg(wi0 + p), wj = __ldcg(wj0 + p);
        const float si[4] = {sc * wi.x, sc * wi.y, sc * wi.z, sc * wi.w};
        const float vj[4] = {wj.x, wj.y, wj.z, wj.w};
#pragma unroll
        for (int i = 0; i < 4; i++)
#pragma unroll
          for (int j = 0; j < 4; j++) a[0][i][j] += si[i] * vj[j];
        if (two) {
          const float4 xi = __ldcg(wi1 + p), xj = __ldcg(wj1 + p);
          const float ti[4] = {sc * xi.x, sc * xi.y, sc * xi.z, sc * xi.w};
          const float uj[4] = {xj.x, xj.y, xj.z, xj.w};
#pragma unroll
          for (int i = 0; i < 4; i++)
#pragma unroll
            for (int j = 0; j < 4; j++) a[1][i][j] += ti[i] * uj[j];
        }
      }
      {
        float d[32];
#pragma unroll
        for (int qq = 0; qq < 2; qq++)
#pragma unroll
          for (int i = 0; i < 4; i++)
#pragma unroll
            for (int j = 0; j < 4; j++) d[qq * 16 + i * 4 + j] = a[qq][i][j];
        static_for<0, 5>([&](auto sc) {
          constexpr int st2 = decltype(sc)::value, hstep = 16 >> st2, m = 16 >> st2;
          const bool up = (lane & m) != 0;
#pragma unroll
          for (int k = 0; k < hstep; k++) d[k] = (up ? d[k + hstep] : d[k]) + __shfl_xor_sync(0xffffffffu, up ? d[k] : d[k + hstep], m);
        });
        S.red[warp][lane] = (double)d[0];
      }
      __syncthreads();
      if (tid < 32) {
        const bool own = tid < 16 || two;
        double d = 0.0;
        for (int wv = 0; wv < nwarps; wv++) d += S.red[wv][tid];
        const int idx = nH + (tid < 16 ? tile0 : tile1) * 16 + (tid & 15);
        if (own) {
          R[idx] = d;
          if (xch) xchg_push(W.xc, idx, d);
          else if (RH) RH[idx] = d;
        }
      }
      __syncthreads();
    }
  }
  if (xch) {
    phase_d(1);
    if (tid < 32) {
      for (int tile0 = vcta; tile0 < W.ntiles; tile0 += 2 * ncta) {
        const int tile1 = tile0 + ncta;
        const bool own = tid < 16 || tile1 < W.ntiles;
        const int idx = nH + (tid < 16 ? tile0 : tile1) * 16 + (tid & 15);
        const double d = xchg_pull_sum_lanes(W.xc, idx, own ? R[idx] : 0.0, own, ok);
        if (own) {
          R[idx] = d;
          if (RH) RH[idx] = d;
        }
      }
    }
  }
  if (!__syncthreads_and(ok) && tid == 0) {
    R[nH + W.ntiles * 16 + 7] = 1.0;
    if (RH) RH[nH + W.ntiles * 16 + 7] = 1.0;
  }
}

template <int P> struct FusedCfgOf { static constexpr int LPR = (P == 16) ? 4 : 1, TPB = (P == 16) ? 448 : 224; };

template <int P, bool MARG>
__global__ void __launch_bounds__(FusedCfgOf<P>::TPB, 1)
    ba_fused_kernel(const __grid_constant__ BAWinDev W, const __grid_constant__ BAIter it) {
  constexpr int LPR = FusedCfgOf<P>::LPR;
  extern __shared__ __align__(16) unsigned char smem_raw[];
  FusedSmem<P, LPR>& S = *reinterpret_cast<FusedSmem<P, LPR>*>(smem_raw);
#pragma unroll 1
  for (int chunk = blockIdx.x; chunk < W.nchunks; chunk += gridDim.x) fused_chunk<P, LPR, MARG>(W, it, S, chunk);
  const bool ok = grid_barrier(W.bar, W.bar_target);
  fused_reduce<P, LPR>(W, S, ok, blockIdx.x, gridDim.x);
}

template <int P>
__global__ void __launch_bounds__(FusedCfgOf<P>::TPB, P == 32 ? 2 : 1)
    ba_fused_batch_kernel(const BAWinDev* __restrict__ gW, const BAIter* __restrict__ gIt, const __grid_constant__ BABatchHdr hdr) {
  constexpr int LPR = FusedCfgOf<P>::LPR;
  extern __shared__ __align__(16) unsigned char smem_raw[];
  FusedSmem<P, LPR>& S = *reinterpret_cast<FusedSmem<P, LPR>*>(smem_raw);
#pragma unroll 1
  for (int item = blockIdx.x; item < hdr.total; item += gridDim.x) {
    int w = 0;
    while (w + 1 < hdr.B && item >= hdr.prefix[w + 1]) w++;
    fused_chunk<P, LPR, false>(gW[w], gIt[w], S, item - hdr.prefix[w]);
  }
  const bool ok = grid_barrier(hdr.bar, hdr.bar_target);
#pragma unroll 1
  for (int w = 0; w < hdr.B; w++) fused_reduce<P, LPR>(gW[w], S, ok, (int)((blockIdx.x + (unsigned)w * 41u) % gridDim.x), gridDim.x);
}

struct FusedCfg { bool done = false; int max_ctas = 0; };
static std::mutex g_cfg_mutex;

template <int P, bool MARG>
static cudaError_t launch_cfg(BAWinDev& W, const BAIter& it, cudaStream_t s, unsigned* bar_count) {
  static FusedCfg cfg[64];
  constexpr int TPB = FusedCfgOf<P>::TPB;
  int dev = 0;
  cudaError_t e = cudaGetDevice(&dev);
  if (e != cudaSuccess) return e;
  const int smem = (int)sizeof(FusedSmem<P, FusedCfgOf<P>::LPR>);
  const int threads = TPB;
  int max_ctas;
  {
    std::lock_guard<std::mutex> lk(g_cfg_mutex);
    FusedCfg& c = cfg[dev & 63];
    if (!c.done) {
      e = cudaFuncSetAttribute(ba_fused_kernel<P, MARG>, cudaFuncAttributeMaxDynamicSharedMemorySize, smem);
      if (e != cudaSuccess) return e;
      int per_sm = 0, sms = 0;
      e = cudaOccupancyMaxActiveBlocksPerMultiprocessor(&per_sm, ba_fused_kernel<P, MARG>, TPB, smem);
      if (e != cudaSuccess) return e;
      e = cudaDeviceGetAttribute(&sms, cudaDevAttrMultiProcessorCount, dev);
      if (e != cudaSuccess) return e;
      c.max_ctas = per_sm * sms;
      c.done = true;
    }
    max_ctas = c.max_ctas;
  }
  const int grid = min(W.nchunks, max_ctas);
  *bar_count += (unsigned)grid;
  W.bar_target = *bar_count;
  void* args[2] = {(void*)&W, (void*)&it};
  return cudaLaunchCooperativeKernel((const void*)ba_fused_kernel<P, MARG>, dim3(grid), dim3(threads), args, (size_t)smem, s);
}

template <int P>
static cudaError_t launch_batch_cfg(const BAWinDev* gW, const BAIter* gIt, BABatchHdr& hdr, int max_nf, cudaStream_t s, unsigned* bar_count) {
  static FusedCfg cfg[64];
  constexpr int TPB = FusedCfgOf<P>::TPB;
  int dev = 0;
  cudaError_t e = cudaGetDevice(&dev);
  if (e != cudaSuccess) return e;
  const int smem = (int)sizeof(FusedSmem<P, FusedCfgOf<P>::LPR>);
  const int threads = TPB;
  (void)max_nf;
  int max_ctas;
  {
    std::lock_guard<std::mutex> lk(g_cfg_mutex);
    FusedCfg& c = cfg[dev & 63];
    if (!c.done) {
      e = cudaFuncSetAttribute(ba_fused_batch_kernel<P>, cudaFuncAttributeMaxDynamicSharedMemorySize, smem);
      if (e != cudaSuccess) return e;
      int per_sm = 0, sms = 0;
      e = cudaOccupancyMaxActiveBlocksPerMultiprocessor(&per_sm, ba_fused_batch_kernel<P>, TPB, smem);
      if (e != cudaSuccess) return e;
      e = cudaDeviceGetAttribute(&sms, cudaDevAttrMultiProcessorCount, dev);
      if (e != cudaSuccess) return e;
      c.max_ctas = per_sm * sms;
      c.done = true;
    }
    max_ctas = c.max_ctas;
  }
  const int grid = min(hdr.total, max_ctas);
  *bar_count += (unsigned)grid;
  hdr.bar_target = *bar_count;
  void* args[3] = {(void*)&gW, (void*)&gIt, (void*)&hdr};
  return cudaLaunchCooperativeKernel((const void*)ba_fused_batch_kernel<P>, dim3(grid), dim3(threads), args, (size_t)smem, s);
}

cudaError_t launch_fused_batch_kernel(int P, const BAWinDev* gW, const BAIter* gIt, BABatchHdr& hdr, int max_nf, cudaStream_t s, unsigned* bar_count) {
  return (P == 32) ? launch_batch_cfg<32>(gW, gIt, hdr, max_nf, s, bar_count) : launch_batch_cfg<16>(gW, gIt, hdr, max_nf, s, bar_count);
}

cudaError_t launch_fused_kernel(BAWinDev& W, const BAIter& it, bool marg, cudaStream_t s, unsigned* bar_count) {
  if (W.P == 32) return marg ? launch_cfg<32, true>(W, it, s, bar_count) : launch_cfg<32, false>(W, it, s, bar_count);
  return marg ? launch_cfg<16, true>(W, it, s, bar_count) : launch_cfg<16, false>(W, it, s, bar_count);
}

}
```

### dm-vio_b200/csrc/ba_handle.h

```cpp
#pragma once
#include "../../include/dmvio_b200.h"
#include "ba_device.cuh"
#include "common_host.h"
#include <cstdint>
#include <vector>

namespace dmv {
cudaError_t launch_fused_kernel(BAWinDev& W, const BAIter& it, bool marg, cudaStream_t s, unsigned* bar_count);
cudaError_t launch_fused_batch_kernel(int P, const BAWinDev* gW, const BAIter* gIt, BABatchHdr& hdr, int max_nf, cudaStream_t s, unsigned* bar_count);
void launch_resub_kernel(const BAWinDev& W, const BAIter& it, int apply, double* sums, cudaStream_t s);
void launch_repack(const float* src, float4* dst, int n, cudaStream_t s);
void launch_make_dI(const float* img, float4* dst, int w, int h, cudaStream_t s);
void launch_l2_flush(float4* buf, size_t n, cudaStream_t s);
}

struct HostUpload {
  dmv::BAWinDev win;
  dmv::BAIter it;
};

using dmv::MAXF; using dmv::XCHG_MAXR; using dmv::BAAdj; using dmv::BAMarg;

struct dmv_ba {
  dmv_ba_config cfg;
  dmv_ba_params prm;
  int device = 0;
  cudaStream_t stream = nullptr;
  cudaEvent_t ev[4] = {nullptr, nullptr, nullptr, nullptr};
  int P = 16;
  bool P_auto = true;
  int sms = 132;
  int mp = 0;
  int nf = 0, npts = 0, nres = 0, nchunks = 0, max_chunks = 0;
  int N = 0, NW = 0, T = 0, ntiles = 0;
  int slots[MAXF];
  float4* d_img[MAXF] = {nullptr};
  float* d_stage_img = nullptr;
  BAAdj* d_adj = nullptr;
  float2* d_uv = nullptr;
  float* d_idepth[2] = {nullptr, nullptr};
  int id_cur = 0, id_bak = 0;
  bool zero_alias = false;
  float *d_idepth_zero = nullptr, *d_color = nullptr, *d_weights = nullptr, *d_priorF = nullptr;
  uint8_t* d_st_in = nullptr;
  float* d_en_in = nullptr;
  uint8_t* d_st_new[2] = {nullptr, nullptr};
  float *d_en_new[2] = {nullptr, nullptr}, *d_en_wo[2] = {nullptr, nullptr}, *d_cpt[2] = {nullptr, nullptr}, *d_jpjd[2] = {nullptr, nullptr},
        *d_pout[2] = {nullptr, nullptr};
  double* d_result[2] = {nullptr, nullptr};
  float* d_step = nullptr;
  double* d_part = nullptr;
  float4* d_wg = nullptr;
  float* d_hdig = nullptr;
  float* d_hdi_solve = nullptr;
  int hdi_solve_n = 0;
  unsigned int* d_bar = nullptr;
  unsigned int bar_count = 0;
  double* d_resub_sums = nullptr;
  float4* d_flush = nullptr;
  size_t flush_n = 0;
  HostUpload* h_up = nullptr;
  BAAdj* h_adj = nullptr;
  double* h_result[2] = {nullptr, nullptr};
  float* h_scratch = nullptr;
  float* h_en_newest = nullptr;
  bool en_newest_valid = false;
  size_t scratch_floats = 0;
  int host_start[MAXF + 1];
  int chunk_beg[MAXF + 1];
  std::vector<int> host_of_point;
  std::vector<int> res_slot;
  std::vector<uint8_t> h_st_in;
  std::vector<float> h_en_in;
  bool st_in_clean = false;
  bool no_zero_copy = false;
  bool timing = false;
  int tent = 0;
  bool have_tentative = false, have_committed = false, have_adj = false, have_state = false;
  long long launches = 0;
  float last_ms[4] = {0, 0, 0, 0};
  void* nccl_comm = nullptr;
  int nranks = 1, rank = 0;
  BAMarg* d_marg = nullptr;
  uint8_t* d_marg_mask = nullptr;
  float* d_marg_rtz = nullptr;
  double* d_marg_result = nullptr;
  double* h_marg_result = nullptr;
  float* d_act = nullptr;
  float* h_act = nullptr;
  int act_cap = 0;
  void* xchg_own = nullptr;
  void* xchg_map[XCHG_MAXR] = {nullptr};
  int xchg_pitch = 0;
  bool xchg_on = false;
  unsigned int xchg_seq = 0;
};


#define CK(call)                                                                                   \
  do {                                                                                             \
    cudaError_t _e = (call);                                                                       \
    if (_e != cudaSuccess) return dmv::set_error(DMV_ERR_CUDA, "%s failed: %s", #call, cudaGetErrorString(_e)); \
  } while (0)

#define DMV_INTERNAL extern "C" __attribute__((visibility("hidden")))
DMV_INTERNAL int dmv_ba_fill_descriptor(dmv_ba* b);
DMV_INTERNAL void dmv_ba_next_exchange(dmv_ba* b);
DMV_INTERNAL int dmv_ba_enqueue_exchange(dmv_ba* b);
DMV_INTERNAL void dmv_ba_stage_x(dmv_ba* b, const double* x);
DMV_INTERNAL int dmv_ba_check_ready(dmv_ba* b);
DMV_INTERNAL int dmv_ba_stage_state(dmv_ba* b, const dmv_ba_state* st);
DMV_INTERNAL int dmv_ba_finish_linearize(dmv_ba* b, dmv_ba_lin_result* out, double sums[3]);
```

### include/dmvio_b200_bench.h

```cpp
#ifndef DMVIO_B200_BENCH_H
#define DMVIO_B200_BENCH_H
#include "dmvio_b200.h"
#ifdef __cplusplus
extern "C" {
#endif

int dmv_ba_bench_device(dmv_ba* ba, const double* x, int iters, int flush_l2, float* ms_per_iter, float* ms_kernel);
int dmv_ba_bench_e2e(dmv_ba* ba, const double* x, const dmv_ba_state* st, int iters, double* ms_per_iter);

int dmv_ba_batch_bench(dmv_ba_batch* batch, dmv_ba* const* handles, int n, const double* const* x, const dmv_ba_state* const* st, int iters,
                       double* e2e_ms_per_iter, double* kernel_ms_per_iter);

#ifdef __cplusplus
}
#endif
#endif
```

Baseline: 463.8 million.

## Add per-phase clock probes and tune fused kernel barrier, prior staging, resub reduction

Adds a clocked variant of the fused BA kernel with a phase-stamp benchmark API. Alongside it come several unrelated speed tweaks. The grid barrier now uses a release-reduction instead of fence plus atomic, and per-point priors are staged into shared memory via cp.async. The have_x idepth update splits the 8 target frames across 4 lanes and combines them with shuffles instead of each lane looping over all frames. The reduce phase reverses CTA assignment and takes a single-pass unrolled path for short chunk ranges. These target barrier latency, redundant global loads and tail reduction cost, at the price of more shared memory and extra template instantiations.

```diff
diff --git a/dm-vio_b200/capi.py b/dm-vio_b200/capi.py
--- a/dm-vio_b200/capi.py
+++ b/dm-vio_b200/capi.py
@@ -122,7 +122,7 @@
     "dmv_ba_set_window", "dmv_ba_set_points", "dmv_ba_set_residuals", "dmv_ba_set_adjoints", "dmv_ba_set_state", "dmv_ba_linearize",
     "dmv_ba_get_residual_outputs", "dmv_ba_get_target_energies", "dmv_ba_apply_res", "dmv_ba_accumulate", "dmv_ba_get_point_outputs", "dmv_ba_get_solve_HdiF",
     "dmv_ba_resubstitute", "dmv_ba_backup_points", "dmv_ba_restore_points", "dmv_ba_get_idepth", "dmv_ba_gn_step", "dmv_nccl_unique_id",
-    "dmv_ba_comm_init", "dmv_ba_activate_points", "dmv_ba_marginalize_points", "dmv_ba_drop_residuals", "dmv_ba_reset_oob", "dmv_ba_p2p_export", "dmv_ba_p2p_import", "dmv_ba_last_timing", "dmv_ba_bench_device", "dmv_ba_kernel_launch_count", "dmv_ba_io_bytes", "dmv_ba_set_timing", "dmv_ba_bench_e2e",
+    "dmv_ba_comm_init", "dmv_ba_activate_points", "dmv_ba_marginalize_points", "dmv_ba_drop_residuals", "dmv_ba_reset_oob", "dmv_ba_p2p_export", "dmv_ba_p2p_import", "dmv_ba_last_timing", "dmv_ba_bench_device", "dmv_ba_bench_phases", "dmv_ba_kernel_launch_count", "dmv_ba_io_bytes", "dmv_ba_set_timing", "dmv_ba_bench_e2e",
     "dmv_ba_batch_create", "dmv_ba_batch_destroy", "dmv_ba_batch_gn_step", "dmv_ba_batch_set_timing", "dmv_ba_batch_last_kernel_ms", "dmv_ba_batch_bench",
     "dmv_ct_create", "dmv_ct_destroy", "dmv_ct_set_K", "dmv_ct_set_ref", "dmv_ct_make_coarse_depth", "dmv_ct_get_ref", "dmv_ct_upload_new", "dmv_ct_upload_new_image", "dmv_ct_set_huber",
     "dmv_ci_create", "dmv_ci_destroy", "dmv_ci_set_K", "dmv_ci_upload_first", "dmv_ci_upload_new", "dmv_ci_set_points", "dmv_ci_calc_res_and_gs", "dmv_ci_kernel_launch_count",
@@ -170,6 +170,7 @@
         L.dmv_ba_p2p_import.argtypes = [vp, C.c_int, C.c_int, vp]
         L.dmv_ba_last_timing.argtypes = [vp, f32p]
         L.dmv_ba_bench_device.argtypes = [vp, vp, C.c_int, C.c_int, C.POINTER(C.c_float), C.POINTER(C.c_float)]
+        L.dmv_ba_bench_phases.argtypes = [vp, vp, C.c_int, C.c_int, C.c_int, vp, C.POINTER(C.c_int), f32p]
         L.dmv_ba_kernel_launch_count.argtypes = [vp, C.POINTER(C.c_longlong)]
         L.dmv_ba_set_timing.argtypes = [vp, C.c_int]
         L.dmv_ba_bench_e2e.argtypes = [vp, vp, C.POINTER(BAState), C.c_int, C.POINTER(C.c_double)]
@@ -366,6 +367,14 @@
         check(self.L.dmv_ba_bench_device(self.h, _p(xx), iters, int(flush_l2), C.byref(a), C.byref(b)))
         return a.value, b.value
 
+    def bench_phases(self, x=None, iters=100, flush_l2=True, max_ctas=1024):
+        st = np.zeros((iters, max_ctas, 9), np.uint64)
+        ms = np.zeros(iters, np.float32)
+        n = C.c_int(0)
+        xx = _c(x, np.float64)
+        check(self.L.dmv_ba_bench_phases(self.h, _p(xx), iters, int(flush_l2), max_ctas, st.ctypes.data, C.byref(n), ms))
+        return st[:, :n.value], ms
+
     def launch_count(self):
         n = C.c_longlong(0)
         check(self.L.dmv_ba_kernel_launch_count(self.h, C.byref(n)))
diff --git a/dm-vio_b200/csrc/ba_bench.cu b/dm-vio_b200/csrc/ba_bench.cu
--- a/dm-vio_b200/csrc/ba_bench.cu
+++ b/dm-vio_b200/csrc/ba_bench.cu
@@ -6,7 +6,8 @@
 
 extern "C" {
 
-int dmv_ba_bench_device(dmv_ba* b, const double* x, int iters, int flush_l2, float* ms_per_iter, float* ms_kernel) {
+static int bench_loop(dmv_ba* b, const double* x, int iters, int flush_l2, std::vector<float>& ms, std::vector<float>& ms_k,
+                      unsigned long long* clk, int clk_rows, int* grid) {
   int rc = dmv_ba_check_ready(b);
   if (rc != DMV_OK) return rc;
   if (iters < 1 || iters > 4096) return set_error(DMV_ERR_INVALID, "iters out of range");
@@ -26,7 +27,8 @@
     dmv_ba_next_exchange(b);
     HostUpload& U = *b->h_up;
     CK(cudaEventRecord(e[3 * i], b->stream));
-    CK(launch_fused_kernel(U.win, U.it, false, b->stream, &b->bar_count));
+    if (clk) CK(launch_fused_kernel_clocked(U.win, U.it, b->stream, &b->bar_count, clk + (size_t)i * clk_rows * FUSED_NCLK, grid));
+    else CK(launch_fused_kernel(U.win, U.it, false, b->stream, &b->bar_count));
     CK(cudaEventRecord(e[3 * i + 1], b->stream));
     if (b->nccl_comm && !b->xchg_on) {
       rc = dmv_ba_enqueue_exchange(b);
@@ -37,19 +39,53 @@
   }
   CK(cudaGetLastError());
   CK(cudaStreamSynchronize(b->stream));
-  double tot = 0, pk = 0;
+  ms.assign(iters, 0.f);
+  ms_k.assign(iters, 0.f);
   for (int i = 0; i < iters; i++) {
-    float a = 0, c = 0;
-    cudaEventElapsedTime(&c, e[3 * i], e[3 * i + 1]);
-    if (b->nccl_comm && !b->xchg_on) cudaEventElapsedTime(&a, e[3 * i], e[3 * i + 2]);
-    else a = c;
-    tot += a; pk += c;
+    cudaEventElapsedTime(&ms_k[i], e[3 * i], e[3 * i + 1]);
+    if (b->nccl_comm && !b->xchg_on) cudaEventElapsedTime(&ms[i], e[3 * i], e[3 * i + 2]);
+    else ms[i] = ms_k[i];
   }
   for (auto& ev : e) cudaEventDestroy(ev);
+  b->h_up->it.have_x = 0;
+  b->have_tentative = true;
+  return DMV_OK;
+}
+
+int dmv_ba_bench_device(dmv_ba* b, const double* x, int iters, int flush_l2, float* ms_per_iter, float* ms_kernel) {
+  std::vector<float> ms, ms_k;
+  const int rc = bench_loop(b, x, iters, flush_l2, ms, ms_k, nullptr, 0, nullptr);
+  if (rc != DMV_OK) return rc;
+  double tot = 0, pk = 0;
+  for (int i = 0; i < iters; i++) { tot += ms[i]; pk += ms_k[i]; }
   if (ms_per_iter) *ms_per_iter = (float)(tot / iters);
   if (ms_kernel) *ms_kernel = (float)(pk / iters);
-  b->h_up->it.have_x = 0;
-  b->have_tentative = true;
+  return DMV_OK;
+}
+
+int dmv_ba_bench_phases(dmv_ba* b, const double* x, int iters, int flush_l2, int max_ctas, unsigned long long* stamps, int* n_ctas, float* ms_kernel) {
+  if (!b || !stamps || !n_ctas || !ms_kernel || max_ctas < 1) return set_error(DMV_ERR_INVALID, "bad argument");
+  if (iters < 1 || iters > 4096) return set_error(DMV_ERR_INVALID, "iters out of range");
+  int rc = dmv_ba_check_ready(b);
+  if (rc != DMV_OK) return rc;
+  if (b->nccl_comm) return set_error(DMV_ERR_STATE, "the phase clock times the launch alone: no NCCL communicator");
+  rc = dmv_ba_fill_descriptor(b);
+  if (rc != DMV_OK) return rc;
+  if (b->h_up->win.nchunks > max_ctas) return set_error(DMV_ERR_INVALID, "max_ctas below the window's chunk count");
+  const size_t n = (size_t)iters * max_ctas * FUSED_NCLK;
+  CK(cudaSetDevice(b->device));
+  unsigned long long* d_clk = nullptr;
+  CK(cudaMalloc(&d_clk, n * sizeof(unsigned long long)));
+  if (cudaMemset(d_clk, 0, n * sizeof(unsigned long long)) != cudaSuccess) rc = set_error(DMV_ERR_CUDA, "cudaMemset failed");
+  std::vector<float> ms, ms_k;
+  int grid = 0;
+  if (rc == DMV_OK) rc = bench_loop(b, x, iters, flush_l2, ms, ms_k, d_clk, max_ctas, &grid);
+  if (rc == DMV_OK && cudaMemcpy(stamps, d_clk, n * sizeof(unsigned long long), cudaMemcpyDeviceToHost) != cudaSuccess)
+    rc = set_error(DMV_ERR_CUDA, "cudaMemcpy failed");
+  cudaFree(d_clk);
+  if (rc != DMV_OK) return rc;
+  *n_ctas = grid;
+  for (int i = 0; i < iters; i++) ms_kernel[i] = ms_k[i];
   return DMV_OK;
 }
 
diff --git a/dm-vio_b200/csrc/ba_device.cuh b/dm-vio_b200/csrc/ba_device.cuh
--- a/dm-vio_b200/csrc/ba_device.cuh
+++ b/dm-vio_b200/csrc/ba_device.cuh
@@ -12,6 +12,7 @@
 constexpr int TOP_PART = 92;
 __host__ __device__ constexpr int top_off(int r) { return r * TOP_COLS - (r * (r - 1)) / 2; }
 constexpr int RES_NONE = 255, RES_IN = 0, RES_OOB = 1, RES_OUTLIER = 2;
+constexpr int FUSED_NCLK = 9;
 constexpr int ACC_MISC = 8;
 constexpr int PART_SLOT = 168;
 constexpr int PART_CC = MAXF * PART_SLOT;
diff --git a/dm-vio_b200/csrc/ba_fused.cu b/dm-vio_b200/csrc/ba_fused.cu
--- a/dm-vio_b200/csrc/ba_fused.cu
+++ b/dm-vio_b200/csrc/ba_fused.cu
@@ -77,6 +77,7 @@
   float rec[MAXF][16][P];
   float Wv[P][8 * MAXF + 8];
   float hdi[P];
+  float prior[P];
   float id[P], idz[P];
   float misc[16][8];
   double red[16][32];
@@ -106,18 +107,28 @@
   __shared__ int ok_s;
   __syncthreads();
   if (threadIdx.x == 0) {
-    __threadfence();
-    atomicAdd(bar, 1u);
+    asm volatile("red.release.gpu.global.add.u32 [%0], 1;" ::"l"(bar) : "memory");
     int ok = 1;
     const long long t0 = clock64();
     while ((int)(ld_acquire_u32(bar) - target) < 0) {
       if (clock64() - t0 > 200000000ll) { ok = 0; break; }
     }
-    __threadfence();
     ok_s = ok;
   }
   __syncthreads();
   return ok_s != 0;
+}
+
+constexpr int NCLK = FUSED_NCLK;
+template <bool CLK>
+__device__ __forceinline__ void clk_stamp(unsigned long long* clk, int k, unsigned dep = 0u) {
+  if constexpr (CLK) {
+    if (threadIdx.x == 0) {
+      unsigned long long t = 0;
+      asm volatile("{\n\t.reg .pred p;\n\tsetp.ne.u32 p, %1, 0x7fbadbad;\n\t@p mov.u64 %0, %%globaltimer;\n\t}" : "+l"(t) : "r"(dep) : "memory");
+      clk[(size_t)blockIdx.x * NCLK + k] = t;
+    }
+  }
 }
 
 __device__ __forceinline__ void xchg_push(const BAXchg& X, int idx, double v) {
@@ -182,8 +193,8 @@
   return s;
 }
 
-template <int P, int LPR, bool MARG>
-__device__ __forceinline__ void fused_chunk(const BAWinDev& W, const BAIter& it, FusedSmem<P, LPR>& S, const int chunk) {
+template <int P, int LPR, bool MARG, bool CLK = false>
+__device__ __forceinline__ void fused_chunk(const BAWinDev& W, const BAIter& it, FusedSmem<P, LPR>& S, const int chunk, unsigned long long* clk = nullptr) {
   constexpr int LOGP = (P == 32) ? 5 : 4;
   constexpr int NH = FusedSmem<P, LPR>::NH;
   const int nf = W.nf, N = W.N, mp = W.mp;
@@ -196,9 +207,11 @@
   h = min(h, nf - 1);
   const int ch_start = W.host_start[h] + (chunk - W.chunk_beg[h]) * P;
   const int ch_count = min(P, W.host_start[h + 1] - ch_start);
+  clk_stamp<CLK>(clk, 1, (unsigned)ch_count);
 
   for (int i = tid; i < nf * 32; i += nthreads) cp_async16(&S.AhD[i >> 5][(i & 31) * 2], &A->adHost[h * nf + (i >> 5)][(i & 31) * 2]);
   for (int i = tid; i < nf * 4; i += nthreads) cp_async16(&S.dT[i >> 2][(i & 3) * 2], &A->adTdiag[h * nf + (i >> 2)][(i & 3) * 2]);
+  if (tid < ch_count) cp_async4(&S.prior[tid], W.priorF + ch_start + tid);
   asm volatile("cp.async.commit_group;" ::: "memory");
 
   float e_sum = 0.f, rs_step2 = 0.f, rs_nid = 0.f, rs_cnt = 0.f;
@@ -282,6 +295,7 @@
       idz = __ldg(W.idepth_zero + p);
     }
     if (r == 0 && valid) { S.id[pl] = idepth; S.idz[pl] = idz; }
+    clk_stamp<CLK>(clk, 2, __float_as_uint(idepth) ^ __float_as_uint(uv.x) ^ (unsigned)st);
     bool live = (st != RES_NONE) && (st != RES_OOB);
 
     const float Kl0 = (uv.x - cx) * fxi, Kl1 = (uv.y - cy) * fyi;
@@ -364,6 +378,7 @@
       }
       }
     }
+    clk_stamp<CLK>(clk, 3, __float_as_uint(s.JI00));
 
     int newState;
     float newEnergy;
@@ -486,32 +501,35 @@
     const float2 at2 = __ldg(reinterpret_cast<const float2*>(&A->adTdiagF[h * nf + t][q * 2]));
     float idepth, idz;
     if (it.have_x) {
+      static_assert(MAXF == 8, "4 lanes x 2 targets cover the MAXF frame slots");
       const float4 po0 = __ldg(reinterpret_cast<const float4*>(W.c_pout + (size_t)p * 8));
       const float4 po1 = __ldg(reinterpret_cast<const float4*>(W.c_pout + (size_t)p * 8) + 1);
       const float idb = __ldg(W.idepth_backup + p);
-      float b = po1.w - (it.xc[0] * po0.z + it.xc[1] * po0.w + it.xc[2] * po1.x + it.xc[3] * po1.y);
+      int stc[2];
+      float4 a0[2], a1[2];
+#pragma unroll
+      for (int u = 0; u < 2; u++) {
+        const int cs = min(2 * q + u, nf - 1) * mp + p;
+        stc[u] = __ldg(W.c_st + cs);
+        a0[u] = __ldg(reinterpret_cast<const float4*>(W.c_jpjd + (size_t)cs * 8));
+        a1[u] = __ldg(reinterpret_cast<const float4*>(W.c_jpjd + (size_t)cs * 8) + 1);
+      }
+      float bt = 0.f;
       int ngood = 0;
 #pragma unroll
-      for (int t4 = 0; t4 < MAXF; t4 += 4) {
-        int stc[4];
-        float4 a0[4], a1[4];
-#pragma unroll
-        for (int u = 0; u < 4; u++) {
-          const int cs = min(t4 + u, nf - 1) * mp + p;
-          stc[u] = __ldg(W.c_st + cs);
-          a0[u] = __ldg(reinterpret_cast<const float4*>(W.c_jpjd + (size_t)cs * 8));
-          a1[u] = __ldg(reinterpret_cast<const float4*>(W.c_jpjd + (size_t)cs * 8) + 1);
-        }
-#pragma unroll
-        for (int u = 0; u < 4; u++) {
-          const int tt = t4 + u;
-          const bool good = tt < nf && tt != h && stc[u] == RES_IN;
-          const float* xa = it.xAd[h * nf + min(tt, nf - 1)];
-          const float dot = xa[0] * a0[u].x + xa[1] * a0[u].y + xa[2] * a0[u].z + xa[3] * a0[u].w + xa[4] * a1[u].x + xa[5] * a1[u].y + xa[6] * a1[u].z + xa[7] * a1[u].w;
-          b -= good ? dot : 0.f;
-          ngood += good;
-        }
-      }
+      for (int u = 0; u < 2; u++) {
+        const int tt = 2 * q + u;
+        const bool good = tt < nf && tt != h && stc[u] == RES_IN;
+        const float* xa = it.xAd[h * nf + min(tt, nf - 1)];
+        const float dot = xa[0] * a0[u].x + xa[1] * a0[u].y + xa[2] * a0[u].z + xa[3] * a0[u].w + xa[4] * a1[u].x + xa[5] * a1[u].y + xa[6] * a1[u].z + xa[7] * a1[u].w;
+        bt += good ? dot : 0.f;
+        ngood += good;
+      }
+      bt += __shfl_xor_sync(0xffffffffu, bt, 1);
+      bt += __shfl_xor_sync(0xffffffffu, bt, 2);
+      ngood += __shfl_xor_sync(0xffffffffu, ngood, 1);
+      ngood += __shfl_xor_sync(0xffffffffu, ngood, 2);
+      const float b = (po1.w - (it.xc[0] * po0.z + it.xc[1] * po0.w + it.xc[2] * po1.x + it.xc[3] * po1.y)) - bt;
       const float step = ngood > 0 ? -b * po1.z : 0.f;
       idepth = idb + step;
       idz = idepth;
@@ -525,6 +543,7 @@
       idz = __ldg(W.idepth_zero + p);
     }
     if (r == 0 && q == 0 && valid) { S.id[pl] = idepth; S.idz[pl] = idz; }
+    clk_stamp<CLK>(clk, 2, __float_as_uint(idepth) ^ __float_as_uint(uv.x) ^ (unsigned)st);
     bool live = (st != RES_NONE) && (st != RES_OOB);
 
     const float Kl0 = (uv.x - cx) * fxi, Kl1 = (uv.y - cy) * fyi;
@@ -610,6 +629,7 @@
         sv[16] += hw * hw * (gx * gx + gy * gy);
       }
     }
+    clk_stamp<CLK>(clk, 3, __float_as_uint(sv[0]));
     {
       const unsigned bal = __ballot_sync(0xffffffffu, fin);
       live = live && (((bal >> (lane & ~3)) & 0xfu) == 0xfu);
@@ -753,6 +773,7 @@
   }
   cp_async_wait_all();
   __syncthreads();
+  clk_stamp<CLK>(clk, 4);
 
   for (int e = tid; e < ch_count * 9; e += nthreads) {
     const int k = e / ch_count, pl2 = e - k * ch_count;
@@ -769,7 +790,7 @@
         Hdd += S.rec[tt][8][pl2]; bd += S.rec[tt][9][pl2]; c0 += S.rec[tt][10][pl2]; c1 += S.rec[tt][11][pl2];
         c2 += S.rec[tt][12][pl2]; c3 += S.rec[tt][13][pl2]; ngood += S.rec[tt][14][pl2];
       }
-      float prior = __ldg(W.priorF + p);
+      float prior = S.prior[pl2];
       bool masked = true;
       if constexpr (MARG) { masked = __ldg(W.marg_mask + p) != 0; prior *= __ldg(&W.marg->priorFac); }
       float HdiF = 0.f, bdSum = 0.f, w0 = 0.f, w1 = 0.f, w2 = 0.f, w3 = 0.f;
@@ -854,10 +875,12 @@
     }
   }
   __syncthreads();
-}
-
-template <int P, int LPR>
-__device__ __forceinline__ void fused_reduce(const BAWinDev& W, FusedSmem<P, LPR>& S, bool ok, const int vcta, const int ncta) {
+  clk_stamp<CLK>(clk, 5);
+}
+
+template <int P, int LPR, bool CLK = false>
+__device__ __forceinline__ void fused_reduce(const BAWinDev& W, FusedSmem<P, LPR>& S, bool ok, const int vcta, const int ncta,
+                                             unsigned long long* clk = nullptr) {
   const int nf = W.nf, N = W.N, mp = W.mp;
   const int tid = threadIdx.x, nthreads = blockDim.x;
   const int warp = tid >> 5, lane = tid & 31, nwarps = nthreads >> 5;
@@ -873,8 +896,9 @@
   const int nitems = n_off + n_diag + n_c + n_b + 16 + 4 + (ACC_MISC - 1);
   const int grp = tid >> 4, gl = tid & 15, groups_per_cta = nthreads >> 4;
   const int nch = W.nchunks;
+  const int dcta = ncta - 1 - vcta;
   auto phase_d = [&](const int pass) {
-    for (int base = vcta * groups_per_cta; base < nitems; base += ncta * groups_per_cta) {
+    for (int base = dcta * groups_per_cta; base < nitems; base += ncta * groups_per_cta) {
       const int item = base + grp;
       const bool act = item < nitems;
       int off0 = 0, lo0 = 0, hi0 = act ? nch : 0, off1 = 0, lo1 = 0, hi1 = 0, d0 = 0, d1 = -1;
@@ -908,16 +932,27 @@
       }
       if (pass == 0) {
         double sum = 0.0;
+        if (hi0 - lo0 <= 96 && hi1 - lo1 <= 96) {
+          double v[12];
+#pragma unroll
+          for (int u = 0; u < 12; u++) {
+            const int c = (u < 6 ? lo0 : lo1) + gl + 16 * (u % 6);
+            v[u] = (c < (u < 6 ? hi0 : hi1)) ? __ldcg(part + (u < 6 ? off0 : off1) + (size_t)c * PART_STRIDE) : 0.0;
+          }
+#pragma unroll
+          for (int u = 0; u < 12; u++) sum += v[u];
+        } else {
 #pragma unroll 1
-        for (int seg = 0; seg < 2; seg++) {
-          const int lo = seg ? lo1 : lo0, hi = seg ? hi1 : hi0;
-          const double* __restrict__ src = part + (seg ? off1 : off0);
-          for (int c0 = lo + gl; c0 < hi; c0 += 192) {
-            double v[12];
-#pragma unroll
-            for (int u = 0; u < 12; u++) v[u] = (c0 + 16 * u < hi) ? __ldcg(src + (size_t)(c0 + 16 * u) * PART_STRIDE) : 0.0;
-#pragma unroll
-            for (int u = 0; u < 12; u++) sum += v[u];
+          for (int seg = 0; seg < 2; seg++) {
+            const int lo = seg ? lo1 : lo0, hi = seg ? hi1 : hi0;
+            const double* __restrict__ src = part + (seg ? off1 : off0);
+            for (int c0 = lo + gl; c0 < hi; c0 += 192) {
+              double v[12];
+#pragma unroll
+              for (int u = 0; u < 12; u++) v[u] = (c0 + 16 * u < hi) ? __ldcg(src + (size_t)(c0 + 16 * u) * PART_STRIDE) : 0.0;
+#pragma unroll
+              for (int u = 0; u < 12; u++) sum += v[u];
+            }
           }
         }
         sum += __shfl_xor_sync(0xffffffffu, sum, 8);
@@ -938,6 +973,7 @@
     }
     };
   phase_d(0);
+  clk_stamp<CLK>(clk, 7);
 
   {
     const int T = W.T, npts = W.npts;
@@ -1013,6 +1049,7 @@
       __syncthreads();
     }
   }
+  clk_stamp<CLK>(clk, 8);
   if (xch) {
     phase_d(1);
     if (tid < 32) {
@@ -1036,16 +1073,18 @@
 
 template <int P> struct FusedCfgOf { static constexpr int LPR = (P == 16) ? 4 : 1, TPB = (P == 16) ? 448 : 224; };
 
-template <int P, bool MARG>
+template <int P, bool MARG, bool CLK = false>
 __global__ void __launch_bounds__(FusedCfgOf<P>::TPB, 1)
-    ba_fused_kernel(const __grid_constant__ BAWinDev W, const __grid_constant__ BAIter it) {
+    ba_fused_kernel(const __grid_constant__ BAWinDev W, const __grid_constant__ BAIter it, unsigned long long* clk) {
   constexpr int LPR = FusedCfgOf<P>::LPR;
   extern __shared__ __align__(16) unsigned char smem_raw[];
   FusedSmem<P, LPR>& S = *reinterpret_cast<FusedSmem<P, LPR>*>(smem_raw);
+  clk_stamp<CLK>(clk, 0);
 #pragma unroll 1
-  for (int chunk = blockIdx.x; chunk < W.nchunks; chunk += gridDim.x) fused_chunk<P, LPR, MARG>(W, it, S, chunk);
+  for (int chunk = blockIdx.x; chunk < W.nchunks; chunk += gridDim.x) fused_chunk<P, LPR, MARG, CLK>(W, it, S, chunk, clk);
   const bool ok = grid_barrier(W.bar, W.bar_target);
-  fused_reduce<P, LPR>(W, S, ok, blockIdx.x, gridDim.x);
+  clk_stamp<CLK>(clk, 6);
+  fused_reduce<P, LPR, CLK>(W, S, ok, blockIdx.x, gridDim.x, clk);
 }
 
 template <int P>
@@ -1068,8 +1107,8 @@
 struct FusedCfg { bool done = false; int max_ctas = 0; };
 static std::mutex g_cfg_mutex;
 
-template <int P, bool MARG>
-static cudaError_t launch_cfg(BAWinDev& W, const BAIter& it, cudaStream_t s, unsigned* bar_count) {
+template <int P, bool MARG, bool CLK = false>
+static cudaError_t launch_cfg(BAWinDev& W, const BAIter& it, cudaStream_t s, unsigned* bar_count, unsigned long long* clk = nullptr) {
   static FusedCfg cfg[64];
   constexpr int TPB = FusedCfgOf<P>::TPB;
   int dev = 0;
@@ -1082,10 +1121,10 @@
     std::lock_guard<std::mutex> lk(g_cfg_mutex);
     FusedCfg& c = cfg[dev & 63];
     if (!c.done) {
-      e = cudaFuncSetAttribute(ba_fused_kernel<P, MARG>, cudaFuncAttributeMaxDynamicSharedMemorySize, smem);
+      e = cudaFuncSetAttribute(ba_fused_kernel<P, MARG, CLK>, cudaFuncAttributeMaxDynamicSharedMemorySize, smem);
       if (e != cudaSuccess) return e;
       int per_sm = 0, sms = 0;
-      e = cudaOccupancyMaxActiveBlocksPerMultiprocessor(&per_sm, ba_fused_kernel<P, MARG>, TPB, smem);
+      e = cudaOccupancyMaxActiveBlocksPerMultiprocessor(&per_sm, ba_fused_kernel<P, MARG, CLK>, TPB, smem);
       if (e != cudaSuccess) return e;
       e = cudaDeviceGetAttribute(&sms, cudaDevAttrMultiProcessorCount, dev);
       if (e != cudaSuccess) return e;
@@ -1097,8 +1136,8 @@
   const int grid = min(W.nchunks, max_ctas);
   *bar_count += (unsigned)grid;
   W.bar_target = *bar_count;
-  void* args[2] = {(void*)&W, (void*)&it};
-  return cudaLaunchCooperativeKernel((const void*)ba_fused_kernel<P, MARG>, dim3(grid), dim3(threads), args, (size_t)smem, s);
+  void* args[3] = {(void*)&W, (void*)&it, (void*)&clk};
+  return cudaLaunchCooperativeKernel((const void*)ba_fused_kernel<P, MARG, CLK>, dim3(grid), dim3(threads), args, (size_t)smem, s);
 }
 
 template <int P>
@@ -1144,4 +1183,11 @@
   return marg ? launch_cfg<16, true>(W, it, s, bar_count) : launch_cfg<16, false>(W, it, s, bar_count);
 }
 
-}
+cudaError_t launch_fused_kernel_clocked(BAWinDev& W, const BAIter& it, cudaStream_t s, unsigned* bar_count, unsigned long long* clk, int* grid) {
+  const unsigned before = *bar_count;
+  const cudaError_t e = (W.P == 32) ? launch_cfg<32, false, true>(W, it, s, bar_count, clk) : launch_cfg<16, false, true>(W, it, s, bar_count, clk);
+  *grid = (int)(*bar_count - before);
+  return e;
+}
+
+}
diff --git a/dm-vio_b200/csrc/ba_handle.h b/dm-vio_b200/csrc/ba_handle.h
--- a/dm-vio_b200/csrc/ba_handle.h
+++ b/dm-vio_b200/csrc/ba_handle.h
@@ -7,6 +7,7 @@
 
 namespace dmv {
 cudaError_t launch_fused_kernel(BAWinDev& W, const BAIter& it, bool marg, cudaStream_t s, unsigned* bar_count);
+cudaError_t launch_fused_kernel_clocked(BAWinDev& W, const BAIter& it, cudaStream_t s, unsigned* bar_count, unsigned long long* clk, int* grid);
 cudaError_t launch_fused_batch_kernel(int P, const BAWinDev* gW, const BAIter* gIt, BABatchHdr& hdr, int max_nf, cudaStream_t s, unsigned* bar_count);
 void launch_resub_kernel(const BAWinDev& W, const BAIter& it, int apply, double* sums, cudaStream_t s);
 void launch_repack(const float* src, float4* dst, int n, cudaStream_t s);
diff --git a/include/dmvio_b200_bench.h b/include/dmvio_b200_bench.h
--- a/include/dmvio_b200_bench.h
+++ b/include/dmvio_b200_bench.h
@@ -6,6 +6,7 @@
 #endif
 
 int dmv_ba_bench_device(dmv_ba* ba, const double* x, int iters, int flush_l2, float* ms_per_iter, float* ms_kernel);
+int dmv_ba_bench_phases(dmv_ba* ba, const double* x, int iters, int flush_l2, int max_ctas, unsigned long long* stamps, int* n_ctas, float* ms_kernel);
 int dmv_ba_bench_e2e(dmv_ba* ba, const double* x, const dmv_ba_state* st, int iters, double* ms_per_iter);
 
 int dmv_ba_batch_bench(dmv_ba_batch* batch, dmv_ba* const* handles, int n, const double* const* x, const dmv_ba_state* const* st, int iters,
```

Result: faster. 483.5 million (median of 6 runs) (+4.3%).
